# Keytoyze/Mug-Diffusion

Hardware: NVIDIA H100
Metric: denoising-steps/sec (higher is better)
Workload: dtype f32

## Files before the change

include/mugd.h:

```cpp
#ifndef MUGD_H
#define MUGD_H

#include <stdint.h>

#ifdef __cplusplus
extern "C" {
#endif

#define MUGD_ABI_VERSION 13

typedef struct mugd_handle mugd_handle;
typedef struct mugd_plan mugd_plan;

enum mugd_status {
    MUGD_OK = 0,
    MUGD_ERR_INVALID = 1,
    MUGD_ERR_CUDA = 2,
    MUGD_ERR_NO_DEVICE = 3,
    MUGD_ERR_OOM = 4
};

enum mugd_op_kind {
    MUGD_OP_GEMM = 1,
    MUGD_OP_GROUPNORM = 2,
// ... 66 lines not shown
} mugd_layernorm;

typedef struct mugd_attention {
    const float* q; int64_t ldq;
    const float* k; int64_t ldk;
    const float* v; int64_t ldv;
    float* o; int64_t ldo;
    const float* relpos;
    const float* cgain;
    int32_t B, H, D, Lq, Lk, pos_max; float scale;
} mugd_attention;

typedef struct mugd_s4conv {
    const float* u; int64_t ldu;
    const float* Kt;
    const float* D;
    float* y; int64_t ldy;
    int32_t B, L, H;
} mugd_s4conv;

typedef struct mugd_ddim_update {
    float* x;
    float* x_dup;
    const float* eps;
    const float* noise;
    float* pred_x0;
    const float* coef;
    const int32_t* step;
    int32_t S; int32_t n;
    int32_t cfg; float scale; float temperature;
} mugd_ddim_update;

typedef struct mugd_transpose {
    const float* in; float* out;
    int64_t ldi, ldo; int32_t B, C, L, to_nlc;
} mugd_transpose;

typedef struct mugd_copy2d {
    const float* src; int64_t lds; float* dst; int64_t ldd; int32_t rows, cols;
} mugd_copy2d;

typedef struct mugd_step_advance { int32_t* step; } mugd_step_advance;

typedef struct mugd_notes {
    const float* logits; int64_t ld;
    int32_t* count; int32_t* start_ms; int32_t* end_ms;
    double frame_ms;
    int32_t B, T, K;
} mugd_notes;

typedef struct mugd_embed {
    const float* table;
    const int32_t* ids;
    float* out;
    int32_t B, F, H, n_embed;
} mugd_embed;

typedef struct mugd_tf32_split { float* w_hi; float* lo; int64_t n; } mugd_tf32_split;

typedef struct mugd_posterior {
    const float* params;
    const float* noise;
    float *mean, *logvar, *std, *z;
    float scale;
    int32_t B, Z, L;
} mugd_posterior;

typedef struct mugd_groupnorm_var {
    mugd_groupnorm gn;
    const int32_t* valid;
} mugd_groupnorm_var;

typedef struct mugd_attention_var {
    mugd_attention attn;
    const int32_t* valid;
} mugd_attention_var;

typedef struct mugd_row_mask {
    float* x; int64_t ld;
    const int32_t* valid;
    int32_t B, L, cols, reserved_;
} mugd_row_mask;

typedef struct mugd_op {
    int32_t kind;
    int32_t tag;
    union {
        mugd_gemm gemm; mugd_groupnorm gn; mugd_layernorm ln; mugd_attention attn; mugd_s4conv s4;
        mugd_ddim_update ddim; mugd_transpose tr; mugd_copy2d cp; mugd_step_advance adv; mugd_notes notes;
        mugd_embed embed; mugd_tf32_split split; mugd_posterior post;
        mugd_groupnorm_var gnv; mugd_attention_var attnv; mugd_row_mask mask;
    } u;
} mugd_op;

int  mugd_abi_version(void);
const char* mugd_last_error(void);
int  mugd_create(int device, mugd_handle** out);
void mugd_destroy(mugd_handle* h);
int  mugd_device_info(mugd_handle* h, int32_t* sm_count, int32_t* cc_major, int32_t* cc_minor);
int  mugd_set_gemm_impl(mugd_handle* h, int impl);
int  mugd_set_pdl(int enabled);

int  mugd_op_run(mugd_handle* h, const mugd_op* op, void* stream);

int  mugd_plan_create(mugd_handle* h, const mugd_op* ops, int32_t n_ops, mugd_plan** out);
int  mugd_plan_run(mugd_plan* p, void* stream);
int  mugd_plan_capture(mugd_plan* p, void* stream);
int  mugd_plan_replay(mugd_plan* p, int32_t times, void* stream);
int  mugd_plan_launch_count(mugd_plan* p);
void mugd_plan_destroy(mugd_plan* p);

int  mugd_sample(mugd_plan* eval_plan, const mugd_op* tail, int32_t n_tail, int32_t n_steps, void* stream);

typedef struct mugd_stage {
    float* x; float* x_dup;
    const float* x0;
    const float* mask;
    const float* q_noise;
    const float* q_coef;
    const float* noise;
    float* noise_rows;
    int32_t B, C, L, reserved_;
} mugd_stage;
int  mugd_sample_staged(mugd_plan* eval_plan, const mugd_stage* stage, const mugd_op* tail, int32_t n_tail, int32_t n_steps,
                        void* stream);

typedef struct mugd_plms {
    mugd_ddim_update update;
    const float* eps;
    float* e_prime;
    float* hist;
    float* x_stash;
    int32_t cfg; float scale;
} mugd_plms;
int  mugd_sample_plms(mugd_plan* eval_plan, const mugd_plms* p, int32_t first_step, int32_t n_steps, void* stream);
int  mugd_plms_combine(const mugd_plms* p, int32_t step, int32_t heun, void* stream);

#define MUGD_MAX_STEPS 1000
typedef struct mugd_ddpm {
    float* x; float* x_dup;
    const float* eps;
    float* pred_x0;
    const float* noise;
    const float* coef;
    int32_t* step;
    int32_t T, B, C, L;
    int32_t cfg; float scale;
    int32_t clip;
    int32_t reserved_;
} mugd_ddpm;
int  mugd_sample_ddpm(mugd_plan* eval_plan, const mugd_ddpm* d, int32_t first_step, int32_t n_steps, void* stream);
int  mugd_ddpm_update(const mugd_ddpm* d, void* stream);

typedef struct mugd_dpm {
    float* x; float* x_dup;
    const float* eps;
    float* pred_x0;
    float* ring;
    const float* coef;
    int32_t* step;
    int32_t n, S;
    int32_t cfg; float scale;
} mugd_dpm;
int  mugd_sample_dpm(mugd_plan* eval_plan, const mugd_dpm* d, int32_t first_step, int32_t n_steps, void* stream);
int  mugd_dpm_update(const mugd_dpm* d, void* stream);

typedef struct mugd_dpm_ex {
    mugd_dpm dpm;
    const mugd_stage* stage;
    const int32_t* start;
    const float* order_coef;
    int32_t B, reserved_;
} mugd_dpm_ex;
int  mugd_sample_dpm_ex(mugd_plan* eval_plan, const mugd_dpm_ex* e, int32_t first_step, int32_t n_steps, void* stream);
// ... 130 lines not shown
```

mug_diffusion_b200/bundle.py:

```python
from __future__ import annotations

import argparse
import ctypes as C
import os
from typing import Dict, List, Optional, Tuple

import numpy as np
import torch

from . import lib as L_
from . import seeding
from .engine import OpList
from .runtime import Plan, _ptr
from .sampler import draw_step_noise, q_coef_table


def _save_plan(eng, ops: OpList, regions: List[L_.Region], path: str) -> Plan:
    pl = Plan(eng, ops)
    arr = (L_.Region * len(regions))(*regions)
    L_.check(eng.lib.mugd_plan_save(pl.handle, arr, len(regions), path.encode()), f"plan_save {path}")
    return pl


def export_bundle(model, inp: Dict[str, torch.Tensor], S: int, scale: float, out_dir: str, eta: float = 0.0, temperature: float = 1.0,
                  noise_dropout: float = 0.0, inpaint: Optional[Tuple[torch.Tensor, torch.Tensor]] = None,
                  seeds=None) -> Dict[str, torch.Tensor]:
    from .sampler import DDIMSampler

    os.makedirs(out_dir, exist_ok=True)
    eng = model.engine
    dev = eng.device
    cfg = eng.cfg
    B, Cz, Lz = inp["x_T"].shape
    if seeds is not None:
        if noise_dropout > 0.:
            raise ValueError("a seeded bundle draws no dropout mask")
        seeds = seeding.chart_seeds(seeds, B)
    cfg_on = scale != 1.0
    Beff = 2 * B if cfg_on else B
    sampler = DDIMSampler(model)
    sampler.make_schedule(S, ddim_eta=eta, verbose=False)
    ts = np.flip(sampler.ddim_timesteps)
    total = len(ts)

    with eng.lock:
        sess = eng.session(Beff, Lz, per_sample_t=False)
        dec = eng.decoder_session(B, Lz)
        T = inp["c"].shape[2]
        sess.set_ctx_tokens(T)
        seeded = None if seeds is None else seeding.ChartNoise(seeds, (B, Cz, Lz), dev)
        x_T = inp["x_T"] if seeded is None else seeded.draw(seeding.X_T, 0)
        st = dict(in_x=x_T.to(dev).contiguous(), in_c=inp["c"].to(dev).contiguous(), in_uc=inp["uc"].to(dev).contiguous(),
                  pred=torch.zeros(B * Lz * Cz, device=dev), out_z=torch.zeros(B, Cz, Lz, device=dev),
                  out_logits=torch.zeros(B, cfg.decoder.x_channels, dec.Lout, device=dev))
        w4 = [w.to(dev).contiguous() for w in list(inp["w"])[-cfg.unet.levels:]]
        for i, w in enumerate(w4):
            st[f"in_w{i}"] = w
        has_noise = bool(np.any(np.asarray(sampler.ddim_sigmas) != 0))
        staged = has_noise or inpaint is not None
        shape = (B, Cz, Lz)
        if has_noise:
            st["noise_rows"] = torch.zeros(B * Lz * Cz, device=dev)
            st["in_noise"] = torch.empty((total,) + shape, device=dev)
        if inpaint is not None:
            st["in_x0"] = inpaint[0].to(dev, torch.float32).contiguous()
            st["in_mask"] = inpaint[1].to(dev, torch.float32).expand(shape).contiguous()
            st["in_qnoise"] = torch.empty((total,) + shape, device=dev)
            qcoef = q_coef_table(model, ts)
            qcoef.tofile(os.path.join(out_dir, "stage_coef.bin"))
        randn_rows = {} if seeded is None else dict(seeded=seeded, first_draw=total - 1, draw_stride=-1)
        draw_step_noise(total, shape, st.get("in_x0"), st.get("in_qnoise"), has_noise, st.get("in_noise"), noise_dropout, dev,
                        **randn_rows)
        drawn = {} if seeded is None else {"in_x": (seeding.X_T, 0, 1, 1)}
        if seeded is not None:
            drawn.update({k: (p, total - 1, total, -1) for k, p in (("in_noise", seeding.STEP), ("in_qnoise", seeding.Q)) if k in st})
        sess.set_timestep_table(ts.copy())
        sess.set_ddim_schedule(sampler.ddim_alphas, sampler.ddim_alphas_prev, sampler.ddim_sigmas, sampler.ddim_sqrt_one_minus_alphas)

        tensors: Dict[str, torch.Tensor] = dict(weights=eng.weights, weights_lo=eng.weights_lo, arena=sess.arena_t, emb_table=sess.emb_table, temb=sess.temb,
                                                emb_h1=sess.emb_h1, emb_h2=sess.emb_h2, step=sess.step, coef=sess.coef, ctx=sess.ctx,
                                                tc_ws=eng.tc_ws, tc_counters=eng.tc_counters, dec_arena=dec.arena_t)
        for i, t in enumerate(sess.ctx_kv):
            tensors[f"ctx_kv{i}"] = t
        for i, (_, t) in enumerate(sorted(sess.s4_kt.items())):
            tensors[f"s4_kt{i}"] = t
        tensors.update(st)
        contents = {"weights", "weights_lo", "temb", "coef"} | {k for k in tensors if k.startswith("s4_kt")}
        inputs = {k for k in st if k.startswith("in_")}
        names = list(tensors)
        keep = [n.encode() for n in names]
        regions = [L_.Region(keep[i], _ptr(tensors[n]), tensors[n].numel() * tensors[n].element_size()) for i, n in enumerate(names)]

        tail = sess.ddim_tail(B, total, cfg_on, scale, temperature, _ptr(st["pred"]), _ptr(st["noise_rows"]) if has_noise else 0)
        stage = None
        if staged:
            stage = sess.ddim_stage(B, cfg_on, _ptr(st["noise_rows"]) if has_noise else 0)
            if has_noise:
                stage.noise = _ptr(st["in_noise"])
            if inpaint is not None:
                stage.x0, stage.mask, stage.q_noise = _ptr(st["in_x0"]), _ptr(st["in_mask"]), _ptr(st["in_qnoise"])
                stage.q_coef = qcoef.ctypes.data
        readz = OpList()
        readz.transpose(sess.xin.ptr, _ptr(st["out_z"]), sess.xin.ld, 0, B, Cz, Lz, False)
        dec_in = OpList()
        assert cfg.decoder.scale == 1.0, "bundle export assumes first-stage scale 1 (the shipped config)"
        dec_in.transpose(_ptr(st["out_z"]), dec.zin.ptr, 0, dec.zin.ld, B, cfg.decoder.z_channels, Lz, True)
        dec_out = OpList()
        dec_out.transpose(dec.logits.ptr, _ptr(st["out_logits"]), dec.logits.ld, 0, B, cfg.decoder.x_channels, dec.Lout, False)
        ctx_parts = [(_ptr(st["in_uc"]), B), (_ptr(st["in_c"]), B)] if cfg_on else [(_ptr(st["in_c"]), B)]
        seq = [("emb", sess.timestep_ops(total), "run"), ("ctx", sess.context_ops(ctx_parts, T), "run"),
               ("audio", sess.audio_ops([_ptr(w) for w in w4], cfg_on), "run"), ("loadx", sess.loadx_ops(_ptr(st["in_x"]), B, cfg_on), "run"),
               ("eval", None, "graph"), ("tail", tail, "tail"), ("readz", readz, "run"), ("dec_in", dec_in, "run"), ("dec", None, "graph"),
               ("dec_out", dec_out, "run")]
        plans = {}
        lines = ["mugd_bundle 1", f"# z_length {Lz} batch {B} guidance {scale} steps {total} (S={S})"]
        for n in names:
            t = tensors[n]
            nbytes = t.numel() * t.element_size()
            if (n in contents or n in inputs) and n not in drawn:
                t.detach().cpu().contiguous().numpy().tofile(os.path.join(out_dir, n + ".bin"))
                lines.append(f"region {n} {nbytes} file {n}.bin")
            else:
                lines.append(f"region {n} {nbytes} zero -")
        if seeded is not None:
            seeding.seed_array(seeds).tofile(os.path.join(out_dir, "seeds.bin"))
            lines.append(f"seeds seeds.bin {B}")
            for n, (purpose, first, count, stride) in drawn.items():
                lines.append(f"randn {n} {purpose} {first} {count} {stride} {B} {Cz * Lz}")
        for name, ops, mode in seq:
            path = os.path.join(out_dir, name + ".plan")
            if ops is None:
                pl = sess.plan if name == "eval" else dec.plan
                arr = (L_.Region * len(regions))(*regions)
                L_.check(eng.lib.mugd_plan_save(pl.handle, arr, len(regions), path.encode()), f"plan_save {name}")
            else:
                pl = _save_plan(eng, ops, regions, path)
            plans[name] = pl
            if mode == "tail":
                continue
            if name == "eval" and staged:
                for field in ("x", "x_dup", "x0", "mask", "q_noise", "noise", "noise_rows"):
                    ptr = getattr(stage, field)
                    if ptr:
                        region = next(n for n in names if 0 <= ptr - _ptr(tensors[n]) < tensors[n].numel() * tensors[n].element_size())
                        lines.append(f"stage {field} {region} {ptr - _ptr(tensors[region])}")
                lines.append(f"staged eval.plan tail.plan {total} {'stage_coef.bin' if inpaint is not None else '-'} {B} {Cz} {Lz}")
            elif name == "eval":
                lines.append(f"sample eval.plan tail.plan {total}")
            else:
                lines.append(f"plan {name}.plan {mode}")

        sess.set_step(0)
        for name in ("emb", "ctx", "audio", "loadx"):
            plans[name].run()
        sess.plan.launch(total, tail, stage)
        for name in ("readz", "dec_in"):
            plans[name].run()
        dec.plan.launch()
        plans["dec_out"].run()
        torch.cuda.synchronize()
        for n in ("out_z", "out_logits"):
            st[n].cpu().numpy().tofile(os.path.join(out_dir, n + ".expected.bin"))
            lines.append(f"expect {n} {st[n].numel() * 4} {n}.expected.bin")
        open(os.path.join(out_dir, "manifest.txt"), "w").write("\n".join(lines) + "\n")
        return dict(z=st["out_z"].clone(), logits=st["out_logits"].clone())


def main():
    from . import synth
    from .sampler import MugDiffusionB200
# ... 29 lines not shown
```

mug_diffusion_b200/csrc/api.cu:

```cuda
#include <stdarg.h>
#include <string.h>

#include <vector>

#include "common.cuh"

namespace mugd {

static thread_local char g_err[1024] = "";
bool g_use_pdl = true;

void set_error(const char* fmt, ...) {
    va_list ap;
    va_start(ap, fmt);
    vsnprintf(g_err, sizeof(g_err), fmt, ap);
    va_end(ap);
}

}

struct mugd_handle {
    mugd::DeviceInfo dev;
    int default_gemm_impl = MUGD_GEMM_SIMT;
};

struct mugd_plan {
    mugd_handle* h = nullptr;
    std::vector<mugd_op> ops;
    cudaGraph_t graph = nullptr;
    cudaGraphExec_t exec = nullptr;
    int launches = 0;
};

namespace mugd {

const std::vector<mugd_op>& plan_ops(const mugd_plan* p) { return p->ops; }
int plan_from_ops(mugd_handle* h, const mugd_op* ops, int32_t n, mugd_plan** out) { return mugd_plan_create(h, ops, n, out); }

static int dispatch(mugd_handle* h, const mugd_op& op, cudaStream_t st, int* launches, const mugd_gemm* next_tc = nullptr) {
    switch (op.kind) {
        case MUGD_OP_GEMM: return launch_gemm(h->dev, op.u.gemm, h->default_gemm_impl, next_tc, st, launches);
        case MUGD_OP_GROUPNORM: return launch_groupnorm(h->dev, op.u.gn, st, launches);
        case MUGD_OP_LAYERNORM: return launch_layernorm(h->dev, op.u.ln, st, launches);
        case MUGD_OP_ATTENTION: return launch_attention(h->dev, op.u.attn, st, launches);
        case MUGD_OP_S4CONV: return launch_s4conv(h->dev, op.u.s4, st, launches);
        case MUGD_OP_DDIM_UPDATE: return launch_ddim_update(h->dev, op.u.ddim, st, launches);
        case MUGD_OP_TRANSPOSE: return launch_transpose(h->dev, op.u.tr, st, launches);
        case MUGD_OP_COPY2D: return launch_copy2d(h->dev, op.u.cp, st, launches);
        case MUGD_OP_STEP_ADVANCE: return launch_step_advance(h->dev, op.u.adv, st, launches);
        case MUGD_OP_NOTES: return launch_notes(h->dev, op.u.notes, st, launches);
        case MUGD_OP_EMBED: return launch_embed(h->dev, op.u.embed, st, launches);
        case MUGD_OP_TF32_SPLIT: return launch_tf32_split(h->dev, op.u.split, st, launches);
        case MUGD_OP_POSTERIOR: return launch_posterior(h->dev, op.u.post, st, launches);
        case MUGD_OP_GROUPNORM_VAR: return launch_groupnorm_var(h->dev, op.u.gnv, st, launches);
        case MUGD_OP_ATTENTION_VAR: return launch_attention_var(h->dev, op.u.attnv, st, launches);
        case MUGD_OP_ROW_MASK: return launch_row_mask(h->dev, op.u.mask, st, launches);
        default:
            set_error("unknown op kind %d", op.kind);
            return MUGD_ERR_INVALID;
    }
}

template <typename Before, typename After>
static int run_steps(const mugd_plan* eval_plan, int32_t n_steps, int32_t* step, cudaStream_t st, Before before, After after) {
    mugd_step_advance adv;
    adv.step = step;
    for (int32_t k = 0; k < n_steps; ++k) {
        int rc = before(k);
        if (rc != MUGD_OK) return rc;
        MUGD_CHECK_CUDA(cudaGraphLaunch(eval_plan->exec, st));
        if ((rc = after(k)) != MUGD_OK) return rc;
        if (step && (rc = launch_step_advance(eval_plan->h->dev, adv, st, nullptr)) != MUGD_OK) return rc;
    }
    return MUGD_OK;
}

static int no_kernels(int32_t) { return MUGD_OK; }

template <typename Before>
static int run_tail_steps(const mugd_plan* eval_plan, const mugd_op* tail, int32_t n_tail, int32_t n_steps, cudaStream_t st,
                          Before before) {
    return run_steps(eval_plan, n_steps, nullptr, st, before, [&](int32_t) {
        for (int32_t k = 0; k < n_tail; ++k) {
            int rc = dispatch(eval_plan->h, tail[k], st, nullptr);
            if (rc != MUGD_OK) return rc;
        }
        return (int)MUGD_OK;
    });
}

static int run_dpm_steps(const mugd_plan* eval_plan, const mugd_dpm_ex& e, int32_t n_steps, cudaStream_t st) {
    return run_steps(
        eval_plan, n_steps, e.dpm.step, st, [&](int32_t k) { return e.stage ? launch_stage(*e.stage, k, st) : MUGD_OK; },
        [&](int32_t) { return launch_dpm_ex_update(e, st); });
}

static int check_step_range(const char* fn, int32_t first_step, int32_t n_steps, const char* total_name, int32_t total) {
    MUGD_REQUIRE(first_step >= 0 && n_steps >= 0 && (int64_t)first_step + n_steps <= total,
                 "%s: first_step=%d, n_steps=%d outside the %s=%d steps of the request", fn, first_step, n_steps, total_name, total);
    return MUGD_OK;
}

static int check_tail_rows(const char* fn, const char* what, int k, const mugd_ddim_update& d, const float* x, const float* x_dup,
                           int32_t B, int32_t C, int32_t L) {
    const int64_t n = (int64_t)B * C * L;
    MUGD_REQUIRE(d.x == x && d.x_dup == x_dup, "%s: tail op %d updates other rows than the %s's x / x_dup", fn, k, what);
    MUGD_REQUIRE(d.n == n, "%s: tail op %d updates n=%d elements, the %s B*C*L=%lld", fn, k, d.n, what, (long long)n);
    return MUGD_OK;
}

}

using namespace mugd;

extern "C" {

int mugd_abi_version(void) { return MUGD_ABI_VERSION; }

const char* mugd_last_error(void) { return g_err; }

int mugd_create(int device, mugd_handle** out) {
    MUGD_REQUIRE(out, "mugd_create: null out");
    *out = nullptr;
    int n = 0;
    cudaError_t e = cudaGetDeviceCount(&n);
    if (e != cudaSuccess || n <= 0 || device < 0 || device >= n) {
        set_error("mugd_create: no CUDA device %d (count=%d, %s). libmugd has no CPU fallback.", device, n,
                  e == cudaSuccess ? "ok" : cudaGetErrorString(e));
        return MUGD_ERR_NO_DEVICE;
    }
    cudaDeviceProp prop;
    MUGD_CHECK_CUDA(cudaGetDeviceProperties(&prop, device));
    if (prop.major != 9 || prop.minor != 0) {
        set_error("mugd_create: device %d is sm_%d%d; libmugd is built for sm_90a (H100) only", device, prop.major, prop.minor);
        return MUGD_ERR_NO_DEVICE;
    }
    MUGD_CHECK_CUDA(cudaSetDevice(device));
// ... 196 lines not shown
}

int mugd_sample_dpm_ex(mugd_plan* eval_plan, const mugd_dpm_ex* e, int32_t first_step, int32_t n_steps, void* stream) {
    MUGD_REQUIRE(e, "mugd_sample_dpm_ex: null descriptor");
    int rc = check_dpm_ex(*e, n_steps);
    if (rc != MUGD_OK) return rc;
    if ((rc = check_step_range("mugd_sample_dpm_ex", first_step, n_steps, "S", e->dpm.S)) != MUGD_OK) return rc;
    MUGD_REQUIRE(eval_plan && eval_plan->exec, "mugd_sample_dpm_ex: the evaluation plan must be captured (mugd_plan_capture)");
    return run_dpm_steps(eval_plan, *e, n_steps, (cudaStream_t)stream);
}

int mugd_sample_dpm_stop(mugd_plan* eval_plan, const mugd_dpm_stop* e, int32_t first_step, int32_t n_steps, void* stream) {
    MUGD_REQUIRE(e, "mugd_sample_dpm_stop: null descriptor");
    int rc = check_dpm_stop(*e);
    if (rc != MUGD_OK) return rc;
    if ((rc = check_step_range("mugd_sample_dpm_stop", first_step, n_steps, "S", e->dpm.S)) != MUGD_OK) return rc;
    MUGD_REQUIRE(eval_plan && eval_plan->exec, "mugd_sample_dpm_stop: the evaluation plan must be captured (mugd_plan_capture)");
    cudaStream_t st = (cudaStream_t)stream;
    return run_steps(eval_plan, n_steps, e->dpm.step, st, no_kernels, [&](int32_t) { return launch_dpm_stop_update(*e, st); });
}

int mugd_sample_unipc(mugd_plan* eval_plan, const mugd_unipc* u, int32_t first_step, int32_t n_steps, void* stream) {
    MUGD_REQUIRE(u, "mugd_sample_unipc: null descriptor");
    int rc = check_unipc(*u);
    if (rc != MUGD_OK) return rc;
    if ((rc = check_step_range("mugd_sample_unipc", first_step, n_steps, "S", u->dpm.S)) != MUGD_OK) return rc;
    MUGD_REQUIRE(eval_plan && eval_plan->exec, "mugd_sample_unipc: the evaluation plan must be captured (mugd_plan_capture)");
    cudaStream_t st = (cudaStream_t)stream;
    return run_steps(eval_plan, n_steps, u->dpm.step, st, no_kernels, [&](int32_t) { return launch_unipc_update(*u, st); });
}

int mugd_sample_unipc_ex(mugd_plan* eval_plan, const mugd_unipc_ex* e, int32_t first_step, int32_t n_steps, void* stream) {
    MUGD_REQUIRE(e, "mugd_sample_unipc_ex: null descriptor");
    int rc = check_unipc_ex(*e, n_steps);
    if (rc != MUGD_OK) return rc;
    if ((rc = check_step_range("mugd_sample_unipc_ex", first_step, n_steps, "S", e->unipc.dpm.S)) != MUGD_OK) return rc;
    MUGD_REQUIRE(eval_plan && eval_plan->exec, "mugd_sample_unipc_ex: the evaluation plan must be captured (mugd_plan_capture)");
    cudaStream_t st = (cudaStream_t)stream;
    return run_steps(
        eval_plan, n_steps, e->unipc.dpm.step, st, [&](int32_t k) { return e->stage ? launch_stage(*e->stage, k, st) : MUGD_OK; },
        [&](int32_t) { return launch_unipc_ex_update(*e, st); });
}

int mugd_sample_unipc_stop(mugd_plan* eval_plan, const mugd_unipc_stop* e, int32_t first_step, int32_t n_steps, void* stream) {
    MUGD_REQUIRE(e, "mugd_sample_unipc_stop: null descriptor");
    int rc = check_unipc_stop(*e);
    if (rc != MUGD_OK) return rc;
    if ((rc = check_step_range("mugd_sample_unipc_stop", first_step, n_steps, "S", e->unipc.dpm.S)) != MUGD_OK) return rc;
    MUGD_REQUIRE(eval_plan && eval_plan->exec, "mugd_sample_unipc_stop: the evaluation plan must be captured (mugd_plan_capture)");
    cudaStream_t st = (cudaStream_t)stream;
    return run_steps(eval_plan, n_steps, e->unipc.dpm.step, st, no_kernels, [&](int32_t) { return launch_unipc_stop_update(*e, st); });
}

int mugd_sample_join(mugd_plan* eval_plan, const mugd_join* join, const mugd_op* tail, int32_t n_tail, int32_t first_step,
                     int32_t n_steps, void* stream) {
    MUGD_REQUIRE(eval_plan && eval_plan->exec, "mugd_sample_join: the evaluation plan must be captured (mugd_plan_capture)");
    MUGD_REQUIRE(join, "mugd_sample_join: null join");
    MUGD_REQUIRE(n_tail >= 0 && (n_tail == 0 || tail), "mugd_sample_join: bad tail (n_tail=%d)", n_tail);
    const mugd_join& j = *join;
    int rc = check_join(j);
    if (rc != MUGD_OK) return rc;
    const mugd_ddim_update* upd = nullptr;
    for (int k = 0; k < n_tail; ++k) {
        if (tail[k].kind != MUGD_OP_DDIM_UPDATE) continue;
        MUGD_REQUIRE(!upd, "mugd_sample_join: the tail holds more than one DDIM update (op %d)", k);
        upd = &tail[k].u.ddim;
        if ((rc = check_tail_rows("mugd_sample_join", "join", k, *upd, j.x, j.x_dup, j.B, j.C, j.L)) != MUGD_OK) return rc;
        MUGD_REQUIRE(upd->step, "mugd_sample_join: tail op %d has no device step counter", k);
    }
    MUGD_REQUIRE(upd, "mugd_sample_join: the tail holds no DDIM update");
    if ((rc = check_step_range("mugd_sample_join", first_step, n_steps, "S", upd->S)) != MUGD_OK) return rc;
    cudaStream_t st = (cudaStream_t)stream;
    return run_tail_steps(eval_plan, tail, n_tail, n_steps, st, [&](int32_t) { return launch_join(j, upd->step, st); });
}

int mugd_abi_sizes(int32_t* out, int32_t n) {
    MUGD_REQUIRE(out && n >= 13, "abi_sizes: need room for 13 entries");
    out[0] = sizeof(mugd_op); out[1] = sizeof(mugd_gemm); out[2] = sizeof(mugd_groupnorm);
    out[3] = sizeof(mugd_layernorm); out[4] = sizeof(mugd_attention); out[5] = sizeof(mugd_s4conv);
    out[6] = sizeof(mugd_ddim_update); out[7] = sizeof(mugd_transpose); out[8] = sizeof(mugd_copy2d);
    out[9] = sizeof(mugd_notes); out[10] = sizeof(mugd_embed); out[11] = sizeof(mugd_tf32_split);
    out[12] = sizeof(mugd_posterior);
    if (n >= 16) { out[13] = sizeof(mugd_groupnorm_var); out[14] = sizeof(mugd_attention_var); out[15] = sizeof(mugd_row_mask); }
    return MUGD_OK;
}

int mugd_plan_ops(mugd_plan* p, const mugd_op** ops, int32_t* n_ops) {
    MUGD_REQUIRE(p && ops && n_ops, "plan_ops: bad arguments");
    *ops = p->ops.data();
    *n_ops = (int32_t)p->ops.size();
    return MUGD_OK;
}

int mugd_plan_launch_count(mugd_plan* p) { return p ? p->launches : 0; }

void mugd_plan_destroy(mugd_plan* p) {
    if (!p) return;
    if (p->exec) cudaGraphExecDestroy(p->exec);
    if (p->graph) cudaGraphDestroy(p->graph);
    delete p;
}

}
```

mug_diffusion_b200/csrc/common.cuh:

```cuda
#pragma once
#include <cuda_runtime.h>
#include <stdint.h>
#include <stdio.h>
#include <string.h>
#include <string>
#include <utility>

#include "../../include/mugd.h"

#if defined(__CUDA_ARCH__) && (__CUDA_ARCH__ != 900)
#error "libmugd is written for sm_90a (H100) only"
#endif

namespace mugd {

void set_error(const char* fmt, ...);

#define MUGD_CHECK_CUDA(expr)                                                             \
    do {                                                                                  \
        cudaError_t _e = (expr);                                                          \
        if (_e != cudaSuccess) {                                                          \
            ::mugd::set_error("%s:%d %s -> %s", __FILE__, __LINE__, #expr,                \
                              cudaGetErrorString(_e));                                    \
            return MUGD_ERR_CUDA;                                                         \
        }                                                                                 \
    } while (0)

#define MUGD_REQUIRE(cond, ...)                                                           \
    do {                                                                                  \
        if (!(cond)) {                                                                    \
            ::mugd::set_error(__VA_ARGS__);                                               \
            return MUGD_ERR_INVALID;                                                      \
        }                                                                                 \
    } while (0)

struct DeviceInfo {
    int device = 0;
    int sm_count = 132;
    int cc_major = 0, cc_minor = 0;
    int max_smem_optin = 0;
    int tc_single_pass = 0;
    int attention_impl = 1;
    int s4conv_impl = 0;
};

int launch_gemm(const DeviceInfo& dev, const mugd_gemm& g, int default_impl, const mugd_gemm* next, cudaStream_t st, int* launches);
bool gemm_runs_tc(const mugd_gemm& g, int default_impl);
int launch_groupnorm(const DeviceInfo& dev, const mugd_groupnorm& g, cudaStream_t st, int* launches);
int launch_layernorm(const DeviceInfo& dev, const mugd_layernorm& g, cudaStream_t st, int* launches);
int launch_attention(const DeviceInfo& dev, const mugd_attention& a, cudaStream_t st, int* launches);
int launch_s4conv(const DeviceInfo& dev, const mugd_s4conv& s, cudaStream_t st, int* launches);
int launch_ddim_update(const DeviceInfo& dev, const mugd_ddim_update& d, cudaStream_t st, int* launches);
int launch_transpose(const DeviceInfo& dev, const mugd_transpose& t, cudaStream_t st, int* launches);
int launch_copy2d(const DeviceInfo& dev, const mugd_copy2d& c, cudaStream_t st, int* launches);
int launch_step_advance(const DeviceInfo& dev, const mugd_step_advance& a, cudaStream_t st, int* launches);
int launch_notes(const DeviceInfo& dev, const mugd_notes& n, cudaStream_t st, int* launches);
int launch_embed(const DeviceInfo& dev, const mugd_embed& e, cudaStream_t st, int* launches);
int launch_tf32_split(const DeviceInfo& dev, const mugd_tf32_split& s, cudaStream_t st, int* launches);
int launch_posterior(const DeviceInfo& dev, const mugd_posterior& p, cudaStream_t st, int* launches);
int launch_groupnorm_var(const DeviceInfo& dev, const mugd_groupnorm_var& g, cudaStream_t st, int* launches);
int launch_attention_var(const DeviceInfo& dev, const mugd_attention_var& a, cudaStream_t st, int* launches);
int launch_row_mask(const DeviceInfo& dev, const mugd_row_mask& m, cudaStream_t st, int* launches);
int check_stage(const mugd_stage& s, int32_t n_steps);
int launch_stage(const mugd_stage& s, int32_t i, cudaStream_t st);
int check_plms(const mugd_plms& p);
int launch_plms_combine(const mugd_plms& p, int32_t step, int heun, cudaStream_t st);
int check_ddpm(const mugd_ddpm& d);
int launch_ddpm_update(const mugd_ddpm& d, int32_t k, cudaStream_t st);
int check_dpm(const mugd_dpm& d);
int launch_dpm_update(const mugd_dpm& d, cudaStream_t st);
int check_dpm_ex(const mugd_dpm_ex& e, int32_t n_steps);
int launch_dpm_ex_update(const mugd_dpm_ex& e, cudaStream_t st);
int check_dpm_stop(const mugd_dpm_stop& e);
int launch_dpm_stop_update(const mugd_dpm_stop& e, cudaStream_t st);
int check_unipc(const mugd_unipc& u);
int launch_unipc_update(const mugd_unipc& u, cudaStream_t st);
int check_unipc_ex(const mugd_unipc_ex& e, int32_t n_steps);
int launch_unipc_ex_update(const mugd_unipc_ex& e, cudaStream_t st);
int check_unipc_stop(const mugd_unipc_stop& e);
int launch_unipc_stop_update(const mugd_unipc_stop& e, cudaStream_t st);
int check_join(const mugd_join& j);
int launch_join(const mugd_join& j, const int32_t* step, cudaStream_t st);
int launch_gemm_tc(const DeviceInfo& dev, const mugd_gemm& g, const mugd_gemm* next, cudaStream_t st, int* launches);
bool gemm_tc_supported(const mugd_gemm& g);

inline int check_cfg(const char* who, int cfg) {
    MUGD_REQUIRE(cfg == 0 || cfg == 1, "%s: cfg=%d", who, cfg);
    return MUGD_OK;
}
inline int check_scale(const char* who, float scale) {
    MUGD_REQUIRE(isfinite(scale), "%s: scale is not finite", who);
    return MUGD_OK;
}
inline int check_x_dup(const char* who, const float* x_dup, int cfg) {
    MUGD_REQUIRE(!x_dup == !cfg, "%s: x_dup must be given exactly when cfg = 1 (the evaluation reads x in both halves)", who);
    return MUGD_OK;
}
inline int check_tile_grid(const char* who, int32_t B, int32_t C, int32_t L) {
    MUGD_REQUIRE(B > 0 && C > 0 && L > 0 && (int64_t)B * C * L <= INT32_MAX, "%s: bad shape B=%d C=%d L=%d", who, B, C, L);
    MUGD_REQUIRE(B <= 65535 && (C + 31) / 32 <= 65535, "%s: B=%d / C=%d too large for one launch", who, B, C);
    return MUGD_OK;
}

cudaError_t gemm_tc_allow_smem(int bytes);
cudaError_t attention_tc_allow_smem(int bytes);
cudaError_t attention_allow_smem(int bytes);
cudaError_t s4_allow_smem(int bytes);

extern bool g_use_pdl;

#ifdef __CUDACC__
template <typename... KArgs, typename... Args>
inline cudaError_t launch_k(void (*kernel)(KArgs...), dim3 grid, dim3 block, size_t smem, cudaStream_t st, Args&&... args) {
    cudaLaunchConfig_t cfg = {};
    cfg.gridDim = grid;
    cfg.blockDim = block;
    cfg.dynamicSmemBytes = smem;
    cfg.stream = st;
    cudaLaunchAttribute attr[1];
    attr[0].id = cudaLaunchAttributeProgrammaticStreamSerialization;
    attr[0].val.programmaticStreamSerializationAllowed = 1;
    cfg.attrs = attr;
    cfg.numAttrs = g_use_pdl ? 1 : 0;
    return cudaLaunchKernelEx(&cfg, kernel, std::forward<Args>(args)...);
}
template <typename... Kernels>
inline cudaError_t allow_dynamic_smem(int bytes, Kernels... kernels) {
    cudaError_t e = cudaSuccess;
    ((e = (e == cudaSuccess) ? cudaFuncSetAttribute(kernels, cudaFuncAttributeMaxDynamicSharedMemorySize, bytes) : e), ...);
    return e;
}
__device__ __forceinline__ void pdl_wait() { asm volatile("griddepcontrol.wait;" ::: "memory"); }

__device__ __forceinline__ float cfg_eps(const float* eps, int64_t i, int64_t n, int cfg, float scale) {
    if (!cfg) return eps[i];
    const float eu = eps[i], ec = eps[n + i];
    return __fadd_rn(eu, __fmul_rn(scale, __fsub_rn(ec, eu)));
}

__device__ __forceinline__ void load_ncl_tile(float (&tile)[32][33], const float* in, int c0, int l0, int C, int L) {
    const int tx = threadIdx.x & 31, ty = threadIdx.x >> 5;
#pragma unroll
    for (int r = ty; r < 32; r += 8) {
// ... 35 lines not shown
```

mug_diffusion_b200/csrc/gemm_tc.cu:

```cuda
#include "gemm_tc.cuh"

namespace mugd {

template <int BN, int EPI>
__global__ void __launch_bounds__(TC_THREADS, 1)
gemm_tc_kernel(const __grid_constant__ CUtensorMap tmA, const __grid_constant__ CUtensorMap tmA1,
               const __grid_constant__ CUtensorMap tmA2, const __grid_constant__ CUtensorMap tmB, const __grid_constant__ CUtensorMap tmWhi,
               const __grid_constant__ CUtensorMap tmWlo, const __grid_constant__ TcParams p) {
    extern __shared__ uint8_t smem_raw[];
    const uint32_t base = (smem_u32(smem_raw) + 1023u) & ~1023u;
    const TcBars<BN> B(base);
    TC_STAMP(p, 0, blockIdx.x == 0 && blockIdx.y == 0 && blockIdx.z == 0);
    if (threadIdx.x < 32) {
        B.init_parallel((int)threadIdx.x);
    } else if (threadIdx.x < 38) {
        const CUtensorMap* m = threadIdx.x == 32 ? &tmA : threadIdx.x == 33 ? &tmA1 : threadIdx.x == 34 ? &tmA2
                             : threadIdx.x == 35 ? &tmB : threadIdx.x == 36 ? &tmWhi : &tmWlo;
        asm volatile("prefetch.tensormap [%0];" ::"l"(reinterpret_cast<uint64_t>(m)) : "memory");
    }
    __syncthreads();
    TC_STAMP(p, 1, blockIdx.x == 0 && blockIdx.y == 0 && blockIdx.z == 0);
    gemm_tc_tile<BN, EPI>(&tmA, &tmA1, &tmA2, &tmB, &tmWhi, &tmWlo, p, blockIdx.x, blockIdx.y, blockIdx.z, base);
}

template <int BN, int EPI>
__global__ void __launch_bounds__(TC_THREADS)
gemm_tc_reduce_kernel(const __grid_constant__ TcParams p) {
    tc_reduce<BN, EPI>(p, blockIdx.x);
}

#ifdef MUGD_TC_TIMELINE
static long long* g_tc_dbg = nullptr;
#endif
static float g_tc_kstep128 = 0.55f;
static float g_tc_split = 3.0f;
static int g_tc_force_bn = 0;

static bool tc_shape_ok(const mugd_gemm& g) {
    if (!(g.conv_mode == MUGD_CONV_NONE || g.conv_mode == MUGD_CONV_SAME || g.conv_mode == MUGD_CONV_DOWN ||
          g.conv_mode == MUGD_CONV_TAPS)) return false;
    if (g.conv_mode == MUGD_CONV_DOWN && g.Lout < 2) return false;
    if (g.K2 % TC_BK != 0 || (g.K2 > 0 && g.conv_mode == MUGD_CONV_DOWN)) return false;
    return g.K % TC_BK == 0 && g.N >= 16 && g.N % 4 == 0;
}

bool gemm_tc_supported(const mugd_gemm& g) {
    if (!tc_shape_ok(g)) return false;
    if (!g.W_hi || !g.W_lo) return false;
    if (g.lda % 4 != 0 || !aligned16(g.A) || !aligned16(g.W_hi) || !aligned16(g.W_lo)) return false;
    if (g.K2 > 0 && (!g.A2 || g.lda2 % 4 != 0 || !aligned16(g.A2))) return false;
    return true;
}

static int tc_validate_fusions(const mugd_gemm& g) {
    if (g.row_moments)
        MUGD_REQUIRE(g.act == MUGD_ACT_NONE && g.gate == MUGD_GATE_NONE && !g.ln_stats && (reinterpret_cast<uintptr_t>(g.row_moments) & 15u) == 0,
                     "gemm: row_moments needs act == gate == NONE, no folded LayerNorm and a 16-byte aligned buffer");
    if (g.ln_stats) {
        MUGD_REQUIRE(g.ln_colsum && aligned16(g.ln_colsum) && (reinterpret_cast<uintptr_t>(g.ln_stats) & 15u) == 0 && g.taps == 1 && g.K2 == 0 &&
                         g.act == MUGD_ACT_NONE && (g.gate == MUGD_GATE_NONE || g.gate == MUGD_GATE_GEGLU) && !g.rowvec,
                     "gemm: folded LayerNorm needs a single-source Linear with act NONE and gate NONE/GEGLU");
    }
    return MUGD_OK;
}

TcGeometry tc_geometry(const mugd_gemm& g, int sm_count, int forced_split) {
    TcGeometry t = {};
    TcParams::Hot& h = t.hot;
    t.BN = (g.N >= 128) ? 128 : 64;
    if (g.conv_mode == MUGD_CONV_NONE) { h.Lrows = g.M; h.Bs = 1; }
    else { h.Lrows = g.Lout; h.Bs = g.M / g.Lout; }
    if (h.Lrows >= TC_BM) {
        h.box_l = TC_BM; h.box_b = 1;
        h.tiles_per_sample = (h.Lrows + TC_BM - 1) / TC_BM;
        t.gy = h.tiles_per_sample * h.Bs;
    } else {
        h.box_l = h.Lrows;
        h.box_b = TC_BM / h.Lrows;
        if (h.box_b > h.Bs) h.box_b = h.Bs;
        h.tiles_per_sample = 1;
        t.gy = (h.Bs + h.box_b - 1) / h.box_b;
    }
    h.kblocks = g.K / TC_BK;
    h.it_main = g.taps * h.kblocks;
    h.total_it = h.it_main + g.K2 / TC_BK;
    int splits = 1;
    float best = 1e30f;
    static const int cands[2] = {64, 128};
    for (int cand = 0; cand < 2; ++cand) {
        const int bn = cands[cand];
        if (bn > 64 && g.N < bn) continue;
        if (bn == 64 && g.N >= 128 && g_tc_force_bn != 64) continue;
        if (g_tc_force_bn && bn != g_tc_force_bn && !(g_tc_force_bn > g.N && bn == 64)) continue;
        const int gx = (g.N + bn - 1) / bn;
        const int tiles = gx * t.gy;
        const float kstep = bn == 128 ? g_tc_kstep128 : 0.4f;
        const int sp_max = forced_split > 0 ? forced_split : (tiles < sm_count ? 16 : 1);
        for (int sp = forced_split > 0 ? forced_split : 1; sp <= sp_max && sp <= h.total_it; ++sp) {
            const int per = (h.total_it + sp - 1) / sp;
            if (forced_split <= 0 && sp > 1 && per < 2) break;
            if (forced_split <= 0 && sp > 1 && tiles * sp > 2 * sm_count) break;
            const int waves = (tiles * sp + sm_count - 1) / sm_count;
            const float est = waves * (1.0f + kstep * per) + (sp > 1 ? g_tc_split : 0.0f);
            if (est < best - 0.25f) { best = est; splits = sp; t.BN = bn; }
        }
    }
    h.gx = (g.N + t.BN - 1) / t.BN;
    if (splits > h.total_it) splits = h.total_it;
    if (splits < 1) splits = 1;
    h.splits = splits;
    h.it_base = h.total_it / splits;
    h.it_rem = h.total_it % splits;
    h.conv_mode = g.conv_mode;
    h.tap_shift = g.tap_shift;
    h.tap_dilation = g.tap_dilation;
    t.ws_floats = splits > 1 ? (int64_t)h.gx * t.gy * splits * TC_BM * t.BN : 0;
    return t;
}

int tc_plan(const DeviceInfo& dev, const mugd_gemm& g, const mugd_gemm* next, TcPlanned* out) {
    MUGD_REQUIRE(gemm_tc_supported(g), "gemm_tc: unsupported shape/operands");
    int rc = tc_validate_fusions(g);
    if (rc != MUGD_OK) return rc;
    const TcGeometry t = tc_geometry(g, dev.sm_count, g.split_k);
    const TcParams::Hot& h = t.hot;
    if (h.splits > 1) {
        MUGD_REQUIRE(g.workspace, "gemm_tc: split-K needs a workspace");
        MUGD_REQUIRE(g.workspace_bytes >= t.ws_floats * 4, "gemm_tc: workspace too small (%lld < %lld)", (long long)g.workspace_bytes,
                     (long long)t.ws_floats * 4);
    }
    const cuuint32_t a_box[3] = {(cuuint32_t)TC_BK, (cuuint32_t)h.box_l, (cuuint32_t)h.box_b};
    for (int tap = 0; tap < 3; ++tap) {
        if (tap > 0 && g.conv_mode != MUGD_CONV_DOWN) { out->maps[tap] = out->maps[0]; continue; }
        const bool down = g.conv_mode == MUGD_CONV_DOWN;
        const cuuint64_t rows = down ? (cuuint64_t)(h.Lrows - (tap == 2 ? 1 : 0)) : (cuuint64_t)h.Lrows;
        const cuuint64_t sample_rows = down ? (cuuint64_t)g.Lin : (cuuint64_t)h.Lrows;
        const cuuint64_t dims[3] = {(cuuint64_t)g.K, rows, (cuuint64_t)h.Bs};
        const cuuint64_t strides[2] = {(cuuint64_t)g.lda * 4 * (down ? 2 : 1), sample_rows * (cuuint64_t)g.lda * 4};
        rc = encode_f32_tma(&out->maps[tap], g.A + (down ? (int64_t)tap * g.lda : 0), 3, dims, strides, a_box, CU_TENSOR_MAP_L2_PROMOTION_L2_128B,
                            "gemm_tc A");
        if (rc != MUGD_OK) return rc;
    }
    if (g.K2 > 0) {
        const cuuint64_t dims[3] = {(cuuint64_t)g.K2, (cuuint64_t)h.Lrows, (cuuint64_t)h.Bs};
        const cuuint64_t strides[2] = {(cuuint64_t)g.lda2 * 4, (cuuint64_t)h.Lrows * (cuuint64_t)g.lda2 * 4};
        rc = encode_f32_tma(&out->maps[3], g.A2, 3, dims, strides, a_box, CU_TENSOR_MAP_L2_PROMOTION_L2_128B, "gemm_tc A2");
        if (rc != MUGD_OK) return rc;
    } else {
        out->maps[3] = out->maps[0];
    }
    const cuuint64_t ktot = (cuuint64_t)g.taps * g.K + g.K2;
    const cuuint64_t w_dims[2] = {ktot, (cuuint64_t)g.N};
    const cuuint64_t w_strides[1] = {ktot * 4};
    const cuuint32_t w_box[2] = {(cuuint32_t)TC_BK, (cuuint32_t)t.BN};
    for (int w = 0; w < 2; ++w) {
        rc = encode_f32_tma(&out->maps[4 + w], w == 0 ? g.W_hi : g.W_lo, 2, w_dims, w_strides, w_box, CU_TENSOR_MAP_L2_PROMOTION_L2_256B,
                            "gemm_tc W");
        if (rc != MUGD_OK) return rc;
    }
    TcParams& p = out->p;
    memset(&p, 0, sizeof(p));
    p.hot = h;
    p.hot.single_pass = dev.tc_single_pass ? 1 : 0;
    p.g = g;
    p.ws = (float*)g.workspace;
    p.gy = t.gy;
    p.ln_invK = 1.0 / (double)g.K;
    if (next) {
        p.pf_hi = next->W_hi;
        p.pf_lo = p.hot.single_pass ? nullptr : next->W_lo;
        p.pf_bytes = (int64_t)next->N * ((int64_t)next->taps * next->K + next->K2) * 4;
    }
#ifdef MUGD_TC_TIMELINE
    p.dbg = g_tc_dbg;
#endif
    out->BN = t.BN;
    return MUGD_OK;
}

template <int BN, int EPI>
static int tc_launch(const TcPlanned& pl, cudaStream_t st) {
    const TcParams& p = pl.p;
    const TcParams::Hot& h = p.hot;
// ... 108 lines not shown
```

mug_diffusion_b200/csrc/norm.cu:

```cuda
#include "common.cuh"

namespace mugd {

constexpr int GN_THREADS = 256;
constexpr int GN_MAXV = 32;

__device__ __forceinline__ void gn_block_stats(double s, double ss, double inv_n, float eps, float& mean, float& rstd) {
    __shared__ double red[2][GN_THREADS / 32];
    s = warp_sum(s);
    ss = warp_sum(ss);
    const int warp = threadIdx.x >> 5, lane = threadIdx.x & 31;
    if (lane == 0) { red[0][warp] = s; red[1][warp] = ss; }
    __syncthreads();
    double ts = 0.0, tss = 0.0;
#pragma unroll
    for (int w = 0; w < GN_THREADS / 32; ++w) { ts += red[0][w]; tss += red[1][w]; }
    const double m = ts * inv_n;
    const double var = tss * inv_n - m * m;
    const float v = fmaxf((float)var, 0.f) + eps;
    float r = rsqrtf(v);
    r = r * (1.5f - 0.5f * v * r * r);
    mean = (float)m;
    rstd = r;
}

template <int NV>
__device__ __forceinline__ void gn_reg_body(const float* __restrict__ x, int64_t ldx, float* __restrict__ y, int64_t ldy,
                                            const float* __restrict__ gamma, const float* __restrict__ beta,
                                            int L, int Lv, int C, int G, float eps, int silu) {
    const int g = blockIdx.x, b = blockIdx.y;
    const int cg = C / G;
    const int q = cg >> 2;
    const int total = Lv * q;
    const double inv_n = 1.0 / ((double)Lv * cg);
    const float* xb = x + (int64_t)b * L * ldx + (int64_t)g * cg;
    float* yb = y + (int64_t)b * L * ldy + (int64_t)g * cg;
    float4 v[NV];
#pragma unroll
    for (int u = 0; u < NV; ++u) {
        const int i = (int)threadIdx.x + u * GN_THREADS;
        v[u] = make_float4(0.f, 0.f, 0.f, 0.f);
        if (i < total) {
            const int row = i / q, qq = i - row * q;
            v[u] = ld_f4(xb + (int64_t)row * ldx + qq * 4);
        }
    }
    double s = 0.0, ss = 0.0;
#pragma unroll
    for (int u = 0; u < NV; ++u) {
        s += (double)v[u].x + (double)v[u].y + (double)v[u].z + (double)v[u].w;
        ss += (double)v[u].x * v[u].x + (double)v[u].y * v[u].y + (double)v[u].z * v[u].z + (double)v[u].w * v[u].w;
    }
    const float* gm = gamma + g * cg;
    const float* bt = beta + g * cg;
    constexpr bool PRE = NV <= 8;
    float4 gav[PRE ? NV : 1], bev[PRE ? NV : 1];
    if constexpr (PRE) {
#pragma unroll
        for (int u = 0; u < NV; ++u) {
            const int i = (int)threadIdx.x + u * GN_THREADS;
            const int qq = i < total ? i % q : 0;
            gav[u] = ld_f4(gm + qq * 4);
            bev[u] = ld_f4(bt + qq * 4);
        }
    }
    float mean, rstd;
    gn_block_stats(s, ss, inv_n, eps, mean, rstd);
#pragma unroll
    for (int u = 0; u < NV; ++u) {
        const int i = (int)threadIdx.x + u * GN_THREADS;
        if (i < total) {
            const int row = i / q, qq = i - row * q;
            float4 ga, be;
            if constexpr (PRE) { ga = gav[u]; be = bev[u]; }
            else { ga = ld_f4(gm + qq * 4); be = ld_f4(bt + qq * 4); }
            float4 o;
            o.x = (v[u].x - mean) * rstd * ga.x + be.x;
            o.y = (v[u].y - mean) * rstd * ga.y + be.y;
            o.z = (v[u].z - mean) * rstd * ga.z + be.z;
            o.w = (v[u].w - mean) * rstd * ga.w + be.w;
            if (silu) { o.x = silu_f(o.x); o.y = silu_f(o.y); o.z = silu_f(o.z); o.w = silu_f(o.w); }
            st_f4(yb + (int64_t)row * ldy + qq * 4, o);
        }
    }
}

template <int NV>
__global__ void __launch_bounds__(GN_THREADS)
groupnorm_silu_reg_kernel(const float* __restrict__ x, int64_t ldx, float* __restrict__ y, int64_t ldy,
                          const float* __restrict__ gamma, const float* __restrict__ beta,
                          int L, int C, int G, float eps, int silu) {
    pdl_wait();
    gn_reg_body<NV>(x, ldx, y, ldy, gamma, beta, L, L, C, G, eps, silu);
}

__device__ __forceinline__ void gn_body(const float* __restrict__ x, int64_t ldx, float* __restrict__ y, int64_t ldy,
                                        const float* __restrict__ gamma, const float* __restrict__ beta,
                                        int L, int Lv, int C, int G, float eps, int silu) {
    const int g = blockIdx.x, b = blockIdx.y;
    const int cg = C / G;
    const int q = cg >> 2;
    const int total = Lv * q;
    const double inv_n = 1.0 / ((double)Lv * cg);
    const float* xb = x + (int64_t)b * L * ldx + (int64_t)g * cg;
    float* yb = y + (int64_t)b * L * ldy + (int64_t)g * cg;

    double s = 0.0, ss = 0.0;
    for (int i = threadIdx.x; i < total; i += GN_THREADS) {
        const int row = i / q, qq = i - row * q;
        const float4 v = ld_f4(xb + (int64_t)row * ldx + qq * 4);
        s += (double)v.x + (double)v.y + (double)v.z + (double)v.w;
        ss += (double)v.x * v.x + (double)v.y * v.y + (double)v.z * v.z + (double)v.w * v.w;
    }
    float mean, rstd;
    gn_block_stats(s, ss, inv_n, eps, mean, rstd);
    const float* gm = gamma + g * cg;
    const float* bt = beta + g * cg;
    for (int i = threadIdx.x; i < total; i += GN_THREADS) {
        const int row = i / q, qq = i - row * q;
        const float4 v = ld_f4(xb + (int64_t)row * ldx + qq * 4);
        const float4 ga = ld_f4(gm + qq * 4);
        const float4 be = ld_f4(bt + qq * 4);
        float4 o;
        o.x = (v.x - mean) * rstd * ga.x + be.x;
        o.y = (v.y - mean) * rstd * ga.y + be.y;
        o.z = (v.z - mean) * rstd * ga.z + be.z;
        o.w = (v.w - mean) * rstd * ga.w + be.w;
        if (silu) { o.x = silu_f(o.x); o.y = silu_f(o.y); o.z = silu_f(o.z); o.w = silu_f(o.w); }
        st_f4(yb + (int64_t)row * ldy + qq * 4, o);
    }
}

__global__ void __launch_bounds__(GN_THREADS)
groupnorm_silu_kernel(const float* __restrict__ x, int64_t ldx, float* __restrict__ y, int64_t ldy,
                      const float* __restrict__ gamma, const float* __restrict__ beta,
                      int L, int C, int G, float eps, int silu) {
    pdl_wait();
    gn_body(x, ldx, y, ldy, gamma, beta, L, L, C, G, eps, silu);
}

__device__ __forceinline__ int gn_valid_rows(const int32_t* valid, int L) { return min(max(valid[blockIdx.y], 0), L); }

__device__ __forceinline__ void gn_zero_tail(float* y, int64_t ldy, int L, int Lv, int C, int G) {
    const int g = blockIdx.x, b = blockIdx.y;
    const int q = (C / G) >> 2;
    float* yb = y + ((int64_t)b * L + Lv) * ldy + (int64_t)g * (C / G);
    const float4 z = make_float4(0.f, 0.f, 0.f, 0.f);
    for (int i = threadIdx.x; i < (L - Lv) * q; i += GN_THREADS) {
        const int row = i / q, qq = i - row * q;
        st_f4(yb + (int64_t)row * ldy + qq * 4, z);
    }
}

template <int NV>
__global__ void __launch_bounds__(GN_THREADS)
groupnorm_silu_reg_var_kernel(const float* __restrict__ x, int64_t ldx, float* __restrict__ y, int64_t ldy,
                              const float* __restrict__ gamma, const float* __restrict__ beta,
                              int L, int C, int G, float eps, int silu, const int32_t* __restrict__ valid) {
    pdl_wait();
    const int Lv = gn_valid_rows(valid, L);
    gn_reg_body<NV>(x, ldx, y, ldy, gamma, beta, L, Lv, C, G, eps, silu);
    gn_zero_tail(y, ldy, L, Lv, C, G);
}

__global__ void __launch_bounds__(GN_THREADS)
groupnorm_silu_var_kernel(const float* __restrict__ x, int64_t ldx, float* __restrict__ y, int64_t ldy,
                          const float* __restrict__ gamma, const float* __restrict__ beta,
                          int L, int C, int G, float eps, int silu, const int32_t* __restrict__ valid) {
    pdl_wait();
    const int Lv = gn_valid_rows(valid, L);
    gn_body(x, ldx, y, ldy, gamma, beta, L, Lv, C, G, eps, silu);
    gn_zero_tail(y, ldy, L, Lv, C, G);
}

static int check_groupnorm(const mugd_groupnorm& g) {
    MUGD_REQUIRE(g.B > 0 && g.L > 0 && g.C > 0 && g.G > 0, "groupnorm: empty shape B=%d L=%d C=%d G=%d", g.B, g.L, g.C, g.G);
    MUGD_REQUIRE(g.C % g.G == 0 && (g.C / g.G) % 4 == 0, "groupnorm: C/G must be a multiple of 4 (C=%d G=%d)", g.C, g.G);
    MUGD_REQUIRE(g.ldx % 4 == 0 && g.ldy % 4 == 0 && aligned16(g.x) && aligned16(g.y) && aligned16(g.gamma) && aligned16(g.beta),
                 "groupnorm: operands must be 16-byte aligned with ld %% 4 == 0");
    MUGD_REQUIRE(g.ldx >= g.C && g.ldy >= g.C, "groupnorm: leading dimension smaller than C");
    return MUGD_OK;
}

int launch_groupnorm(const DeviceInfo&, const mugd_groupnorm& g, cudaStream_t st, int* launches) {
    const int rc = check_groupnorm(g);
    if (rc != MUGD_OK) return rc;
    dim3 grid(g.G, g.B);
    const int per_thread = (g.L * (g.C / g.G / 4) + GN_THREADS - 1) / GN_THREADS;
#define GN_GO(K) MUGD_CHECK_CUDA(launch_k(K, grid, dim3(GN_THREADS), 0, st, g.x, g.ldx, g.y, g.ldy, g.gamma, g.beta, g.L, g.C, g.G, g.eps, g.silu))
    if (per_thread <= 2) GN_GO(groupnorm_silu_reg_kernel<2>);
    else if (per_thread <= 4) GN_GO(groupnorm_silu_reg_kernel<4>);
    else if (per_thread <= 8) GN_GO(groupnorm_silu_reg_kernel<8>);
    else if (per_thread <= 16) GN_GO(groupnorm_silu_reg_kernel<16>);
    else if (per_thread <= GN_MAXV) GN_GO(groupnorm_silu_reg_kernel<GN_MAXV>);
    else GN_GO(groupnorm_silu_kernel);
#undef GN_GO
    if (launches) *launches += 1;
    return MUGD_OK;
}

int launch_groupnorm_var(const DeviceInfo&, const mugd_groupnorm_var& v, cudaStream_t st, int* launches) {
    const mugd_groupnorm& g = v.gn;
    int rc = check_groupnorm(g);
    if (rc != MUGD_OK) return rc;
    MUGD_REQUIRE(v.valid, "groupnorm_var: valid lengths missing");
    dim3 grid(g.G, g.B);
    const int per_thread = (g.L * (g.C / g.G / 4) + GN_THREADS - 1) / GN_THREADS;
#define GN_GO(K) MUGD_CHECK_CUDA(launch_k(K, grid, dim3(GN_THREADS), 0, st, g.x, g.ldx, g.y, g.ldy, g.gamma, g.beta, g.L, g.C, g.G, g.eps, g.silu, v.valid))
    if (per_thread <= 2) GN_GO(groupnorm_silu_reg_var_kernel<2>);
    else if (per_thread <= 4) GN_GO(groupnorm_silu_reg_var_kernel<4>);
    else if (per_thread <= 8) GN_GO(groupnorm_silu_reg_var_kernel<8>);
    else if (per_thread <= 16) GN_GO(groupnorm_silu_reg_var_kernel<16>);
    else if (per_thread <= GN_MAXV) GN_GO(groupnorm_silu_reg_var_kernel<GN_MAXV>);
    else GN_GO(groupnorm_silu_var_kernel);
#undef GN_GO
    if (launches) *launches += 1;
    return MUGD_OK;
}

constexpr int LN_WARPS = 8;
constexpr int LN_MAXQ = 8;

__global__ void __launch_bounds__(LN_WARPS * 32)
layernorm_kernel(const float* __restrict__ x, int64_t ldx, float* __restrict__ y, int64_t ldy,
                 const float* __restrict__ gamma, const float* __restrict__ beta, int rows, int C, float eps) {
    pdl_wait();
    const int row = blockIdx.x * LN_WARPS + (threadIdx.x >> 5);
    if (row >= rows) return;
    const int lane = threadIdx.x & 31;
    const int nq = C >> 2;
    const float* xr = x + (int64_t)row * ldx;
    float4 v[LN_MAXQ];
    float s = 0.f;
#pragma unroll
    for (int i = 0; i < LN_MAXQ; ++i) {
        const int qi = lane + i * 32;
        if (qi < nq) {
            v[i] = ld_f4(xr + qi * 4);
            s += (v[i].x + v[i].y) + (v[i].z + v[i].w);
        } else {
            v[i] = make_float4(0.f, 0.f, 0.f, 0.f);
        }
    }
    const float mean = warp_sum(s) / (float)C;
    float ss = 0.f;
#pragma unroll
    for (int i = 0; i < LN_MAXQ; ++i) {
        const int qi = lane + i * 32;
        if (qi < nq) {
            const float a = v[i].x - mean, b = v[i].y - mean, c = v[i].z - mean, d = v[i].w - mean;
            ss += (a * a + b * b) + (c * c + d * d);
        }
    }
    const float rstd = rsqrtf(warp_sum(ss) / (float)C + eps);
    float* yr = y + (int64_t)row * ldy;
#pragma unroll
    for (int i = 0; i < LN_MAXQ; ++i) {
        const int qi = lane + i * 32;
        if (qi < nq) {
            const float4 ga = ld_f4(gamma + qi * 4), be = ld_f4(beta + qi * 4);
            float4 o;
            o.x = (v[i].x - mean) * rstd * ga.x + be.x;
            o.y = (v[i].y - mean) * rstd * ga.y + be.y;
            o.z = (v[i].z - mean) * rstd * ga.z + be.z;
            o.w = (v[i].w - mean) * rstd * ga.w + be.w;
            st_f4(yr + qi * 4, o);
        }
    }
}

int launch_layernorm(const DeviceInfo&, const mugd_layernorm& g, cudaStream_t st, int* launches) {
    MUGD_REQUIRE(g.rows > 0 && g.C > 0, "layernorm: empty shape");
    MUGD_REQUIRE(g.C % 4 == 0 && g.C <= LN_MAXQ * 128, "layernorm: C=%d must be a multiple of 4 and <= %d", g.C, LN_MAXQ * 128);
    MUGD_REQUIRE(g.ldx % 4 == 0 && g.ldy % 4 == 0 && aligned16(g.x) && aligned16(g.y) && aligned16(g.gamma) && aligned16(g.beta),
                 "layernorm: operands must be 16-byte aligned with ld %% 4 == 0");
    MUGD_REQUIRE(g.ldx >= g.C && g.ldy >= g.C, "layernorm: leading dimension smaller than C");
    const int blocks = (g.rows + LN_WARPS - 1) / LN_WARPS;
    MUGD_CHECK_CUDA(launch_k(layernorm_kernel, dim3(blocks), dim3(LN_WARPS * 32), 0, st, g.x, g.ldx, g.y, g.ldy, g.gamma, g.beta, g.rows,
                             g.C, g.eps));
    if (launches) *launches += 1;
    return MUGD_OK;
}

}
```

mug_diffusion_b200/engine.py:

```python
from __future__ import annotations

import ctypes as C
from dataclasses import dataclass
from typing import Dict, List, Optional, Sequence, Tuple

import numpy as np
import torch

from . import lib as L_
from .config import DecoderConfig, EncoderConfig, ModelConfig, UNetConfig
from .dpm_solver import MAX_STEPS
from .netspec import RES_LAYERS, Block, decoder_layout, encoder_layout, unet_layout
from .packer import WeightBlob, pack_model

GN_EPS = 1e-6
LN_EPS = 1e-5
CTX_TOKENS_MAX = 64


@dataclass
class View:
    ptr: int
    ld: int
    rows: int
    cols: int

    def c(self, c0: int, c1: int) -> "View":
        assert 0 <= c0 < c1 <= self.cols, (c0, c1, self.cols)
        return View(self.ptr + 4 * c0, self.ld, self.rows, c1 - c0)

    def r(self, r0: int, r1: int) -> "View":
        assert 0 <= r0 < r1 <= self.rows
        return View(self.ptr + 4 * r0 * self.ld, self.ld, r1 - r0, self.cols)


class Arena:

    def __init__(self, base: int = 0, capacity: Optional[int] = None):
        self.base = base
        self.capacity = capacity
        self.top = 0
        self.high = 0

    def alloc(self, rows: int, cols: int) -> View:
        n = rows * cols * 4
        start = (self.top + 255) // 256 * 256
        self.top = start + n
        self.high = max(self.high, self.top)
        if self.capacity is not None:
            assert self.top <= self.capacity, "arena overflow"
        return View(self.base + start, cols, rows, cols)

    def mark(self) -> int:
        return self.top

    def release(self, mark: int):
        self.top = mark


class OpList:
    def __init__(self, tc_map: Optional[Dict[int, Tuple[int, int]]] = None, valid: Optional[Dict[int, int]] = None):
        self.ops: List[L_.Op] = []
        self.tc_map = tc_map or {}
        self.valid = valid or {}

    def add(self, kind: int, desc, tag: int = 0):
        self.ops.append(L_.make_op(kind, desc, tag))

    def array(self):
        arr = (L_.Op * len(self.ops))(*self.ops)
        return arr

    def gemm(self, A: View, W: int, N: int, K: int, out: View, *, bias: int = 0, taps: int = 1,
             mode: int = L_.CONV_NONE, Lin: int = 0, Lout: int = 0, act: int = L_.ACT_NONE,
             gate: int = L_.GATE_NONE, residual: Optional[View] = None, rowvec: int = 0,
             rowvec_b_stride: int = 0, rowvec_step_stride: int = 0, step: int = 0, impl: int = L_.GEMM_AUTO,
             W_hi: int = 0, W_lo: int = 0, split_k: int = 0, tap_shift: int = 0, dilation: int = 1, tag: int = 0,
             A2: Optional[View] = None, ln: Optional[Tuple[int, int, float]] = None) -> int:
        g = L_.Gemm()
        M = out.rows
        g.A, g.lda = A.ptr, A.ld
        if not W_hi and W in self.tc_map:
            W_hi, W_lo = self.tc_map[W]
        g.W, g.W_hi, g.W_lo, g.bias = W, W_hi or None, W_lo or None, bias or None
        g.split_k = split_k
        g.tap_shift = tap_shift
        g.tap_dilation = dilation
        g.rowvec, g.rowvec_b_stride, g.rowvec_step_stride = rowvec or None, rowvec_b_stride, rowvec_step_stride
        g.step = step or None
        if residual is not None:
            g.residual, g.ldr = residual.ptr, residual.ld
        if A2 is not None:
            assert A2.rows == out.rows, (A2.rows, out.rows)
            g.A2, g.lda2, g.K2 = A2.ptr, A2.ld, A2.cols
        g.C, g.ldc = out.ptr, out.ld
        g.M, g.N, g.K = M, N, K
        g.taps, g.conv_mode = taps, mode
        g.Lout = Lout or M
        g.Lin = Lin or g.Lout
        g.act, g.gate, g.impl = act, gate, impl
        if ln is not None:
            g.ln_stats, g.ln_colsum, g.ln_eps = ln[0], ln[1], float(ln[2])
        nout = N // 2 if gate else N
        assert out.cols == nout, (out.cols, nout)
        assert A.cols == K, (A.cols, K)
        self.add(L_.OP_GEMM, g, tag)
        return len(self.ops) - 1

    def can_deliver_row_moments(self, i: int) -> bool:
        op = self.ops[i]
        if op.kind != L_.OP_GEMM:
            return False
        g = op.u.gemm
        tc = bool(g.W_hi) and g.K % 32 == 0 and g.K2 % 32 == 0 and g.N >= 16 and g.impl != L_.GEMM_SIMT and g.conv_mode != L_.CONV_UP
        return tc and g.act == L_.ACT_NONE and g.gate == L_.GATE_NONE and not g.ln_stats and not g.row_moments

    def groupnorm(self, x: View, y: View, gamma: int, beta: int, B: int, Lrows: int, G: int, silu: bool, tag: int = 0) -> int:
        d = L_.GroupNorm()
        d.x, d.ldx, d.y, d.ldy = x.ptr, x.ld, y.ptr, y.ld
        d.gamma, d.beta = gamma, beta
        d.B, d.L, d.C, d.G = B, Lrows, x.cols, G
        d.eps, d.silu = GN_EPS, int(silu)
        assert x.rows == B * Lrows and y.cols == x.cols
        if Lrows in self.valid:
            v = L_.GroupNormVar()
            v.gn, v.valid = d, self.valid[Lrows]
            self.add(L_.OP_GROUPNORM_VAR, v, tag)
        else:
            self.add(L_.OP_GROUPNORM, d, tag)
        return len(self.ops) - 1

    def row_mask(self, x: View, B: int, Lrows: int, tag: int = 0):
        assert x.rows == B * Lrows
        d = L_.RowMask()
        d.x, d.ld, d.valid = x.ptr, x.ld, self.valid[Lrows]
        d.B, d.L, d.cols = B, Lrows, x.cols
        self.add(L_.OP_ROW_MASK, d, tag)

    def layernorm(self, x: View, y: View, gamma: int, beta: int, tag: int = 0):
        d = L_.LayerNorm()
        d.x, d.ldx, d.y, d.ldy = x.ptr, x.ld, y.ptr, y.ld
        d.gamma, d.beta = gamma, beta
        d.rows, d.C, d.eps = x.rows, x.cols, LN_EPS
        self.add(L_.OP_LAYERNORM, d, tag)
        return len(self.ops) - 1

    def attention(self, q: View, k: View, v: View, o: View, relpos: int, cgain: int, B: int, H: int, Lq: int,
                  Lk: int, pos_max: int, tag: int = 0, self_attn: bool = False):
        d = L_.Attention()
        D = q.cols // H
        d.q, d.ldq, d.k, d.ldk, d.v, d.ldv, d.o, d.ldo = q.ptr, q.ld, k.ptr, k.ld, v.ptr, v.ld, o.ptr, o.ld
        d.relpos, d.cgain = relpos, cgain
        d.B, d.H, d.D, d.Lq, d.Lk, d.pos_max = B, H, D, Lq, Lk, pos_max
        d.scale = float(D) ** -0.5
        if self_attn and Lq in self.valid:
            v = L_.AttentionVar()
            v.attn, v.valid = d, self.valid[Lq]
            self.add(L_.OP_ATTENTION_VAR, v, tag)
        else:
            self.add(L_.OP_ATTENTION, d, tag)

    def s4conv(self, u: View, Kt: int, Dp: int, y: View, B: int, Lrows: int, tag: int = 0):
        d = L_.S4Conv()
        d.u, d.ldu, d.Kt, d.D, d.y, d.ldy = u.ptr, u.ld, Kt, Dp, y.ptr, y.ld
        d.B, d.L, d.H = B, Lrows, u.cols
        self.add(L_.OP_S4CONV, d, tag)

    def transpose(self, inp: int, out: int, ldi: int, ldo: int, B: int, Cc: int, Lrows: int, to_nlc: bool, tag: int = 0):
        d = L_.Transpose()
        d.inp, d.out, d.ldi, d.ldo = inp, out, ldi, ldo
        d.B, d.C, d.L, d.to_nlc = B, Cc, Lrows, int(to_nlc)
        self.add(L_.OP_TRANSPOSE, d, tag)

    def copy2d(self, src: View, dst: View, tag: int = 0):
        d = L_.Copy2D()
        assert src.rows == dst.rows and src.cols == dst.cols
        d.src, d.lds, d.dst, d.ldd, d.rows, d.cols = src.ptr, src.ld, dst.ptr, dst.ld, src.rows, src.cols
        self.add(L_.OP_COPY2D, d, tag)


def emit_upsample_conv(ops: "OpList", blob: WeightBlob, wfn, prefix: str, x: View, out: View, Lin: int, cin: int, cout: int, tag: int):
    idx = []
    if (prefix + "conv.up_even.weight") in blob.entries:
        for parity, name, shift in ((0, "conv.up_even.weight", -1), (1, "conv.up_odd.weight", 0)):
            dst = View(out.ptr + 4 * parity * out.ld, 2 * out.ld, x.rows, out.cols)
            idx.append(ops.gemm(x, wfn(prefix + name), cout, cin, dst, bias=wfn(prefix + "conv.bias"), taps=2, mode=L_.CONV_TAPS,
                                Lin=Lin, Lout=Lin, tap_shift=shift, tag=tag))
    else:
        idx.append(ops.gemm(x, wfn(prefix + "conv.weight"), cout, cin, out, bias=wfn(prefix + "conv.bias"), taps=3, mode=L_.CONV_UP,
                            Lin=Lin, Lout=2 * Lin, tag=tag))
    return idx


def tc_weight_map(blob: WeightBlob, wbase: int, lo_base: Optional[int] = None) -> Dict[int, Tuple[int, int]]:
    if lo_base is None:
        lo_base = wbase + 4 * blob.numel
    return {wbase + 4 * off: (wbase + 4 * off, lo_base + 4 * lo) for _, off, _, lo in blob.tc}


TAG_RES, TAG_ATTN, TAG_S4, TAG_UPDOWN, TAG_IO = 1, 2, 3, 4, 5


def emit_res(ops: OpList, arena: Arena, wfn, b: Block, x: View, out: View, B: int, Lr: int, G: int, **emb):
    norm1, conv1, norm2, conv2, _ = RES_LAYERS[b.kind]
    p = b.prefix
    m = arena.mark()
    t1 = arena.alloc(x.rows, b.cin)
    ops.groupnorm(x, t1, wfn(p + norm1 + "weight"), wfn(p + norm1 + "bias"), B, Lr, G, True, TAG_RES)
    t2 = arena.alloc(x.rows, b.cout)
    ops.gemm(t1, wfn(p + conv1 + "weight"), b.cout, b.cin, t2, bias=wfn(p + conv1 + "bias"), taps=3, mode=L_.CONV_SAME, Lin=Lr, Lout=Lr,
             tag=TAG_RES, **emb)
    t3 = arena.alloc(x.rows, b.cout)
    ops.groupnorm(t2, t3, wfn(p + norm2 + "weight"), wfn(p + norm2 + "bias"), B, Lr, G, True, TAG_RES)
    if b.has_skip_conv:
        ops.gemm(t3, wfn(p + "out_skip.weight"), b.cout, b.cout, out, bias=wfn(p + "out_skip.bias"), taps=3, mode=L_.CONV_SAME,
                 Lin=Lr, Lout=Lr, A2=x, tag=TAG_RES)
    else:
        ops.gemm(t3, wfn(p + conv2 + "weight"), b.cout, b.cout, out, bias=wfn(p + conv2 + "bias"), taps=3, mode=L_.CONV_SAME,
                 Lin=Lr, Lout=Lr, residual=x, tag=TAG_RES)
    arena.release(m)


class UNetCompiler:

    def __init__(self, cfg: UNetConfig, blob: WeightBlob, wbase: int, tc_map: Optional[Dict[int, Tuple[int, int]]] = None,
                 prefix: str = "model.unet_model."):
        self.cfg, self.blob, self.wbase, self.prefix = cfg, blob, wbase, prefix
        self.tc_map = tc_weight_map(blob, wbase) if tc_map is None else tc_map
        self.lay = unet_layout(cfg, prefix)

    def w(self, name: str) -> int:
        return self.wbase + 4 * self.blob.offset(name)

    def compile(self, arena: Arena, Beff: int, Lz: int, ext: Dict[str, int], per_sample_t: bool, fold_ln: Optional[bool] = None,
                valid: Optional[Sequence[int]] = None) -> dict:
        cfg = self.cfg
        nlev = cfg.levels
        assert Lz % (1 << (nlev - 1)) == 0 and (Lz >> (nlev - 1)) % 4 == 0, "z_length must be a multiple of 32"
        rows = [Beff * (Lz >> l) for l in range(nlev)]
        lens = [Lz >> l for l in range(nlev)]
        if valid is not None:
            assert len(valid) == nlev, (len(valid), nlev)
        ops = OpList(self.tc_map, None if valid is None else {lens[l]: int(valid[l]) for l in range(nlev)})
        ragged = valid is not None
        mc = cfg.model_channels
        G = cfg.gn_groups
        if fold_ln is None:
            fold_ln = rows[0] < 8192
        fuse_ln = fold_ln and any(k.endswith("qkv_ln.weight") for k in self.blob.entries)

        lvl_of_ds = {1 << l: l for l in range(nlev)}
        ln_rows = sum(3 * rows[lvl_of_ds[b.ds]] for b in self.lay.blocks() if b.kind == "attn")
        stat_doubles = ln_rows * 2 if fuse_ln else 0
        stat_floats = (2 * stat_doubles + 63) // 64 * 64
        live = arena.alloc(1, stat_floats) if fuse_ln else None
        zeros = arena.alloc(1, stat_floats) if fuse_ln else None
        stat_top = [0]

        def stat_alloc(n_doubles: int) -> int:
            o = stat_top[0]
            stat_top[0] += (n_doubles + 1) // 2 * 2
            assert stat_top[0] <= stat_doubles, "row-moment block overflow"
            return live.ptr + 8 * o

        if fuse_ln:
            ops.copy2d(zeros, live, TAG_IO)

        xin = arena.alloc(rows[0], cfg.in_channels)
        eps = arena.alloc(rows[0], cfg.out_channels)
        ctx_tokens = ext["ctx_tokens"]
        down_cat = []
        ch = mc
        ch_in_level = []
        for l in range(nlev):
            ch_in_level.append(ch)
            down_cat.append(arena.alloc(rows[l], ch + cfg.audio_channels[l]))
            ch = cfg.channel_mult[l] * mc
        up_blocks = [e for e in self.lay.output if not isinstance(e, tuple)]
        up_cat: List[View] = []
        up_parts: List[Tuple[int, int, int]] = []
        skip_ch = list(self.lay.skip_channels)
        ch = cfg.channel_mult[-1] * mc
        bi = 0
        for level in reversed(range(nlev)):
            for i in range(cfg.num_res_blocks + 1):
                ich = skip_ch.pop()
                ca = cfg.audio_channels[level] if i == 0 else 0
                up_cat.append(arena.alloc(rows[level], ch + ca + ich))
                up_parts.append((ch, ca, ich))
                assert up_blocks[bi][0].cin == ch + ca + ich, (up_blocks[bi][0].cin, ch, ca, ich)
                ch = cfg.channel_mult[level] * mc
                bi += 1
        n_skips = len(self.lay.skip_channels)
        skip_home: List[View] = [None] * n_skips
        for k in range(n_skips):
            ub = n_skips - 1 - k
            ch_h, ca, ich = up_parts[ub]
            assert ich == self.lay.skip_channels[k]
            skip_home[k] = up_cat[ub].c(ch_h + ca, ch_h + ca + ich)
        audio_slots: List[Tuple[int, View]] = []
        for l in range(nlev):
            audio_slots.append((l, down_cat[l].c(ch_in_level[l], ch_in_level[l] + cfg.audio_channels[l])))
        bi = 0
        for level in reversed(range(nlev)):
            ch_h, ca, ich = up_parts[bi]
            audio_slots.append((level, up_cat[bi].c(ch_h, ch_h + ca)))
            bi += cfg.num_res_blocks + 1

        emb_total = self.blob.meta["emb_total"]
        emb_off = self.blob.meta["emb_offsets"]
        E = ext["emb_table"]
        step = ext["step"]

        gemm = ops.gemm

        def copy(src: View, dst: View, tag: int):
            ops.copy2d(src, dst, tag)

        def mask(x: View, lvl: int, tag: int):
            if ragged:
                ops.row_mask(x, Beff, lens[lvl], tag)

        def groupnorm(x: View, y: View, gamma: int, beta: int, Lr: int, silu: bool, tag: int):
            ops.groupnorm(x, y, gamma, beta, Beff, Lr, G, silu, tag)

        emb_row = dict(rowvec_b_stride=emb_total) if per_sample_t else dict(rowvec_step_stride=emb_total, step=step)
        attn_index = [0]

        def emit_attn(b: Block, x: View, out: View, lvl: int):
            Lr, Cc, H = lens[lvl], b.cin, b.heads
            m = arena.mark()
            p = b.prefix
            t = p + "transformer_blocks.0."
            kv = ext["ctx_kv"][attn_index[0]]
            attn_index[0] += 1
            g = arena.alloc(x.rows, Cc)
            groupnorm(x, g, self.w(p + "norm.weight"), self.w(p + "norm.bias"), Lr, False, TAG_ATTN)
            h0 = arena.alloc(x.rows, Cc)
            i_h0 = gemm(g, self.w(p + "proj_in.weight"), Cc, Cc, h0, bias=self.w(p + "proj_in.bias"), Lout=Lr, tag=TAG_ATTN)

            def normed_linear(src: View, i_src: int, norm: str, lin: str, N: int, dst: View, gate: int = L_.GATE_NONE, has_bias: bool = False):
                if fuse_ln and ops.can_deliver_row_moments(i_src):
                    lv = stat_alloc(src.rows * 2)
                    ops.ops[i_src].u.gemm.row_moments = lv
                    gemm(src, self.w(t + lin + "_ln.weight"), N, Cc, dst, bias=self.w(t + lin + "_ln.bias"), gate=gate, Lout=Lr,
                         ln=(lv, self.w(t + lin + "_ln.colsum"), LN_EPS), tag=TAG_ATTN)
                else:
                    n = arena.alloc(src.rows, Cc)
                    ops.layernorm(src, n, self.w(t + norm + ".weight"), self.w(t + norm + ".bias"), TAG_ATTN)
                    gemm(n, self.w(t + lin + ".weight"), N, Cc, dst, bias=self.w(t + lin + ".bias") if has_bias else 0, gate=gate,
                         Lout=Lr, tag=TAG_ATTN)

            qkv = arena.alloc(x.rows, 3 * Cc)
            normed_linear(h0, i_h0, "norm1", "attn1.qkv", 3 * Cc, qkv)
            ao = arena.alloc(x.rows, Cc)
            ops.attention(qkv.c(0, Cc), qkv.c(Cc, 2 * Cc), qkv.c(2 * Cc, 3 * Cc), ao,
                          self.w(t + "attn1.relative_position_embedding"), self.w(t + "attn1.C_embedding"),
                          Beff, H, Lr, Lr, cfg.pos_max, TAG_ATTN, self_attn=True)
            h1 = arena.alloc(x.rows, Cc)
            i_h1 = gemm(ao, self.w(t + "attn1.to_out.0.weight"), Cc, Cc, h1, bias=self.w(t + "attn1.to_out.0.bias"),
                        residual=h0, Lout=Lr, tag=TAG_ATTN)
            q2 = arena.alloc(x.rows, Cc)
            normed_linear(h1, i_h1, "norm2", "attn2.to_q", Cc, q2)
            ops.attention(q2, kv.c(0, Cc), kv.c(Cc, 2 * Cc), ao,
                          self.w(t + "attn2.relative_position_embedding"), self.w(t + "attn2.C_embedding"),
                          Beff, H, Lr, ctx_tokens, cfg.pos_max, TAG_ATTN)
            h2 = h0
            i_h2 = gemm(ao, self.w(t + "attn2.to_out.0.weight"), Cc, Cc, h2, bias=self.w(t + "attn2.to_out.0.bias"),
                        residual=h1, Lout=Lr, tag=TAG_ATTN)
            ff = arena.alloc(x.rows, 4 * Cc)
            normed_linear(h2, i_h2, "norm3", "ff.net.0.proj", 8 * Cc, ff, gate=L_.GATE_GEGLU, has_bias=True)
            gemm(ff, self.w(p + "ff_out.weight"), Cc, 4 * Cc, out, bias=self.w(p + "ff_out.bias"), residual=x, Lout=Lr,
                 A2=h2, tag=TAG_ATTN)
            arena.release(m)

        def emit_s4(b: Block, x: View, out: View, lvl: int):
            Lr, Hc = lens[lvl], b.cin
            m = arena.mark()
            p = b.prefix
            s_ = p + "s4_model."
            g = arena.alloc(x.rows, Hc)
            groupnorm(x, g, self.w(p + "norm.weight"), self.w(p + "norm.bias"), Lr, False, TAG_S4)
            y = arena.alloc(x.rows, Hc)
            ops.s4conv(g, ext["s4_kt"][p].ptr, self.w(s_ + "D"), y, Beff, Lr, TAG_S4)
            z = g
            gemm(y, self.w(s_ + "output_linear.0.weight"), 2 * Hc, Hc, z, bias=self.w(s_ + "output_linear.0.bias"),
                 gate=L_.GATE_GLU, Lout=Lr, tag=TAG_S4)
            mask(z, lvl, TAG_S4)
            gemm(z, self.w(p + "out_layer.weight"), Hc, Hc, out, bias=self.w(p + "out_layer.bias"), taps=3,
                 mode=L_.CONV_SAME, Lin=Lr, Lout=Lr, residual=x, tag=TAG_S4)
            arena.release(m)

        def run_blocks(blocks: List[Block], x: View, final_out: Optional[View], lvl: int) -> Tuple[View, int]:
            cur = x
            for j, b in enumerate(blocks):
                last = j == len(blocks) - 1
                if b.kind == "up":
                    tgt_rows = rows[lvl - 1]
                    out = final_out if (last and final_out is not None) else arena.alloc(tgt_rows, b.cout)
                    mask(cur, lvl, TAG_UPDOWN)
                    emit_upsample_conv(ops, self.blob, self.w, b.prefix, cur, out, lens[lvl], b.cin, b.cout, TAG_UPDOWN)
                    lvl -= 1
                    cur = out
                    continue
                out = final_out if (last and final_out is not None) else arena.alloc(cur.rows, b.cout)
                if b.kind == "res":
                    emit_res(ops, arena, self.w, b, cur, out, Beff, lens[lvl], G, rowvec=E + 4 * emb_off[b.prefix], **emb_row)
                elif b.kind == "attn":
                    emit_attn(b, cur, out, lvl)
                elif b.kind == "s4":
                    emit_s4(b, cur, out, lvl)
                else:
                    raise ValueError(b.kind)
                cur = out
            return cur, lvl

        if ragged:
            mask(xin, 0, TAG_IO)
            for l, view in audio_slots:
                mask(view, l, TAG_IO)

        k = 0
        lvl = 0
        h: Optional[View] = None
        for entry in self.lay.input:
            if isinstance(entry, tuple):
                h = down_cat[lvl]
                continue
            b0 = entry[0]
            if b0.kind == "conv_in":
                dst = down_cat[0].c(0, mc)
                gemm(xin, self.w(b0.prefix + "weight"), b0.cout, b0.cin, dst, bias=self.w(b0.prefix + "bias"), taps=3,
                     mode=L_.CONV_SAME, Lin=lens[0], Lout=lens[0], tag=TAG_IO)
                copy(dst, skip_home[k], TAG_IO)
                k += 1
                h = dst
            elif b0.kind == "down":
                dst = down_cat[lvl + 1].c(0, b0.cout)
                mask(h, lvl, TAG_UPDOWN)
                gemm(h, self.w(b0.prefix + "conv.weight"), b0.cout, b0.cin, dst, bias=self.w(b0.prefix + "conv.bias"),
                     taps=3, mode=L_.CONV_DOWN, Lin=lens[lvl], Lout=lens[lvl + 1], tag=TAG_UPDOWN)
                copy(dst, skip_home[k], TAG_UPDOWN)
                k += 1
                lvl += 1
                h = dst
            else:
                h, lvl = run_blocks(entry, h, skip_home[k], lvl)
                k += 1
        assert k == n_skips and lvl == nlev - 1

        h, lvl = run_blocks(self.lay.middle, h, up_cat[0].c(0, up_parts[0][0]), lvl)

        ub = 0
        final = arena.alloc(rows[0], mc)
        for entry in self.lay.output:
            if isinstance(entry, tuple):
                continue
            if ub + 1 < len(up_cat):
                nxt = up_cat[ub + 1].c(0, up_parts[ub + 1][0])
            else:
                nxt = final
            h, lvl = run_blocks(entry, up_cat[ub], nxt, lvl)
            ub += 1
        assert lvl == 0

        ob = self.lay.out
        m = arena.mark()
        t = arena.alloc(rows[0], mc)
        groupnorm(final, t, self.w(ob.prefix + "0.weight"), self.w(ob.prefix + "0.bias"), lens[0], True, TAG_IO)
        gemm(t, self.w(ob.prefix + "2.weight"), ob.cout, ob.cin, eps, bias=self.w(ob.prefix + "2.bias"), taps=3,
             mode=L_.CONV_SAME, Lin=lens[0], Lout=lens[0], tag=TAG_IO)
        arena.release(m)
        return dict(ops=ops, xin=xin, eps=eps, audio_slots=audio_slots, ln_folded=fuse_ln)


class DecoderCompiler:

    def __init__(self, cfg: DecoderConfig, blob: WeightBlob, wbase: int, tc_map: Optional[Dict[int, Tuple[int, int]]] = None,
                 prefix: str = "model.first_stage_model.decoder."):
        self.cfg, self.blob, self.wbase, self.prefix = cfg, blob, wbase, prefix
        self.tc_map = tc_weight_map(blob, wbase) if tc_map is None else tc_map
        self.seq = self.layout(cfg, prefix)

    layout = staticmethod(decoder_layout)

    def w(self, name: str) -> int:
        return self.wbase + 4 * self.blob.offset(name)

    def compile(self, arena: Arena, B: int, Lz: int, valid: Optional[Dict[int, int]] = None) -> dict:
        cfg = self.cfg
        ops = OpList(self.tc_map, None if valid is None else {Lz * m: int(p) for m, p in valid.items()})
        ragged = valid is not None
        G = cfg.num_groups
        first = self.seq[0]
        inp = arena.alloc(B * Lz * first.mul, first.cin)
        cur = inp
        out_view = None
        for b in self.seq:
            Lr = Lz * b.mul
            p = b.prefix
            if ragged and b.kind in ("dec_conv_in", "up", "down"):
                ops.row_mask(cur, B, Lr, TAG_IO if b.kind == "dec_conv_in" else TAG_UPDOWN)
            if b.kind == "dec_conv_in":
                o = arena.alloc(B * Lr, b.cout)
                ops.gemm(cur, self.w(p + "weight"), b.cout, b.cin, o, bias=self.w(p + "bias"), taps=3, mode=L_.CONV_SAME,
                         Lin=Lr, Lout=Lr, tag=TAG_IO)
                cur = o
            elif b.kind == "dec_res":
                o = arena.alloc(B * Lr, b.cout)
                emit_res(ops, arena, self.w, b, cur, o, B, Lr, G)
                cur = o
            elif b.kind == "up":
                o = arena.alloc(B * Lr * 2, b.cout)
                emit_upsample_conv(ops, self.blob, self.w, p, cur, o, Lr, b.cin, b.cout, TAG_UPDOWN)
                cur = o
            elif b.kind == "down":
                o = arena.alloc(B * Lr // 2, b.cout)
                ops.gemm(cur, self.w(p + "conv.weight"), b.cout, b.cin, o, bias=self.w(p + "conv.bias"), taps=3, mode=L_.CONV_DOWN,
                         Lin=Lr, Lout=Lr // 2, tag=TAG_UPDOWN)
                cur = o
            elif b.kind == "dec_out":
                t = arena.alloc(B * Lr, b.cin)
                ops.groupnorm(cur, t, self.w(p + "norm_out.weight"), self.w(p + "norm_out.bias"), B, Lr, G, True, TAG_IO)
                out_view = arena.alloc(B * Lr, b.cout)
                ops.gemm(t, self.w(p + "conv_out.weight"), b.cout, b.cin, out_view, bias=self.w(p + "conv_out.bias"), taps=3,
                         mode=L_.CONV_SAME, Lin=Lr, Lout=Lr, tag=TAG_IO)
                if ragged:
                    ops.row_mask(out_view, B, Lr, TAG_IO)
            else:
                raise ValueError(b.kind)
        return dict(ops=ops, inp=inp, out=out_view, Lout=Lz * self.seq[-1].mul)


class EncoderCompiler(DecoderCompiler):

    def __init__(self, cfg: EncoderConfig, blob: WeightBlob, wbase: int, tc_map: Optional[Dict[int, Tuple[int, int]]] = None,
                 prefix: str = "model.first_stage_model.encoder."):
        super().__init__(cfg, blob, wbase, tc_map, prefix)

    layout = staticmethod(encoder_layout)
```

mug_diffusion_b200/lib.py:

```python
from __future__ import annotations

import ctypes as C
import os
from typing import Optional

HERE = os.path.dirname(os.path.abspath(__file__))
LIB_PATH = os.environ.get("MUGD_LIB") or os.path.join(HERE, "libmugd.so")

(OP_GEMM, OP_GROUPNORM, OP_LAYERNORM, OP_ATTENTION, OP_S4CONV, OP_DDIM_UPDATE, OP_TRANSPOSE, OP_COPY2D, OP_STEP_ADVANCE, OP_NOTES, OP_EMBED,
 OP_TF32_SPLIT, OP_POSTERIOR) = range(1, 14)
OP_GROUPNORM_VAR, OP_ATTENTION_VAR, OP_ROW_MASK = 14, 15, 16
CONV_NONE, CONV_SAME, CONV_DOWN, CONV_UP, CONV_TAPS = range(5)
ACT_NONE, ACT_SILU, ACT_GELU = range(3)
GATE_NONE, GATE_GEGLU, GATE_GLU = range(3)
GEMM_AUTO, GEMM_SIMT, GEMM_TC = range(3)
ABI_VERSION = 13

_f = C.c_void_p


class Gemm(C.Structure):
    _fields_ = [("A", _f), ("lda", C.c_int64), ("W", _f), ("W_hi", _f), ("W_lo", _f), ("bias", _f), ("rowvec", _f),
                ("rowvec_b_stride", C.c_int64), ("rowvec_step_stride", C.c_int64), ("step", _f),
                ("residual", _f), ("ldr", C.c_int64), ("C", _f), ("ldc", C.c_int64),
# ... 49 lines not shown
class StepAdvance(C.Structure):
    _fields_ = [("step", _f)]


class Notes(C.Structure):
    _fields_ = [("logits", _f), ("ld", C.c_int64), ("count", _f), ("start_ms", _f), ("end_ms", _f), ("frame_ms", C.c_double),
                ("B", C.c_int32), ("T", C.c_int32), ("K", C.c_int32)]


class Embed(C.Structure):
    _fields_ = [("table", _f), ("ids", _f), ("out", _f), ("B", C.c_int32), ("F", C.c_int32), ("H", C.c_int32), ("n_embed", C.c_int32)]


class Tf32Split(C.Structure):
    _fields_ = [("w_hi", _f), ("lo", _f), ("n", C.c_int64)]


class Posterior(C.Structure):
    _fields_ = [("params", _f), ("noise", _f), ("mean", _f), ("logvar", _f), ("std", _f), ("z", _f), ("scale", C.c_float),
                ("B", C.c_int32), ("Z", C.c_int32), ("L", C.c_int32)]


class Stage(C.Structure):
    _fields_ = [("x", _f), ("x_dup", _f), ("x0", _f), ("mask", _f), ("q_noise", _f), ("q_coef", _f), ("noise", _f), ("noise_rows", _f),
                ("B", C.c_int32), ("C", C.c_int32), ("L", C.c_int32), ("reserved_", C.c_int32)]


class Plms(C.Structure):
    _fields_ = [("update", DdimUpdate), ("eps", _f), ("e_prime", _f), ("hist", _f), ("x_stash", _f), ("cfg", C.c_int32),
                ("scale", C.c_float)]


class Ddpm(C.Structure):
    _fields_ = [("x", _f), ("x_dup", _f), ("eps", _f), ("pred_x0", _f), ("noise", _f), ("coef", _f), ("step", _f),
                ("T", C.c_int32), ("B", C.c_int32), ("C", C.c_int32), ("L", C.c_int32), ("cfg", C.c_int32), ("scale", C.c_float),
                ("clip", C.c_int32), ("reserved_", C.c_int32)]


class Dpm(C.Structure):
    _fields_ = [("x", _f), ("x_dup", _f), ("eps", _f), ("pred_x0", _f), ("ring", _f), ("coef", _f), ("step", _f),
                ("n", C.c_int32), ("S", C.c_int32), ("cfg", C.c_int32), ("scale", C.c_float)]


class DpmEx(C.Structure):
    _fields_ = [("dpm", Dpm), ("stage", _f), ("start", _f), ("order_coef", _f), ("B", C.c_int32), ("reserved_", C.c_int32)]


class DpmStop(C.Structure):
    _fields_ = [("dpm", Dpm), ("stop", _f), ("B", C.c_int32), ("reserved_", C.c_int32)]


class Unipc(C.Structure):
    _fields_ = [("dpm", Dpm), ("xc", _f), ("corr", _f)]


class UnipcEx(C.Structure):
    _fields_ = [("unipc", Unipc), ("stage", _f), ("start", _f), ("order_coef", _f), ("order_corr", _f), ("B", C.c_int32),
                ("reserved_", C.c_int32)]


class UnipcStop(C.Structure):
    _fields_ = [("unipc", Unipc), ("stop", _f), ("B", C.c_int32), ("reserved_", C.c_int32)]


class QEncode(C.Structure):
    _fields_ = [("x0", _f), ("noise", _f), ("t", _f), ("sqrt_a", _f), ("sqrt_1ma", _f), ("out", _f),
                ("B", C.c_int32), ("C", C.c_int32), ("L", C.c_int32), ("n", C.c_int32)]


class Join(C.Structure):
    _fields_ = [("x", _f), ("x_dup", _f), ("x_latent", _f), ("join", _f),
                ("B", C.c_int32), ("C", C.c_int32), ("L", C.c_int32), ("reserved_", C.c_int32)]


class Normal(C.Structure):
    _fields_ = [("out", _f), ("seeds", _f), ("n", C.c_int64), ("B", C.c_int32), ("purpose", C.c_int32), ("first_draw", C.c_int32),
                ("n_draws", C.c_int32), ("draw_stride", C.c_int32), ("reserved_", C.c_int32)]


class GroupNormVar(C.Structure):
    _fields_ = [("gn", GroupNorm), ("valid", _f)]


class AttentionVar(C.Structure):
    _fields_ = [("attn", Attention), ("valid", _f)]


class RowMask(C.Structure):
    _fields_ = [("x", _f), ("ld", C.c_int64), ("valid", _f), ("B", C.c_int32), ("L", C.c_int32), ("cols", C.c_int32),
                ("reserved_", C.c_int32)]


class _OpU(C.Union):
    _fields_ = [("gemm", Gemm), ("gn", GroupNorm), ("ln", LayerNorm), ("attn", Attention), ("s4", S4Conv),
                ("ddim", DdimUpdate), ("tr", Transpose), ("cp", Copy2D), ("adv", StepAdvance), ("notes", Notes), ("embed", Embed),
                ("split", Tf32Split), ("post", Posterior), ("gnv", GroupNormVar), ("attnv", AttentionVar), ("mask", RowMask)]


class Op(C.Structure):
    _fields_ = [("kind", C.c_int32), ("tag", C.c_int32), ("u", _OpU)]


_KIND_FIELD = {OP_GEMM: "gemm", OP_GROUPNORM: "gn", OP_LAYERNORM: "ln", OP_ATTENTION: "attn", OP_S4CONV: "s4",
               OP_DDIM_UPDATE: "ddim", OP_TRANSPOSE: "tr", OP_COPY2D: "cp", OP_STEP_ADVANCE: "adv", OP_NOTES: "notes", OP_EMBED: "embed", OP_TF32_SPLIT: "split",
               OP_POSTERIOR: "post", OP_GROUPNORM_VAR: "gnv", OP_ATTENTION_VAR: "attnv", OP_ROW_MASK: "mask"}


def make_op(kind: int, desc, tag: int = 0) -> Op:
    op = Op()
    op.kind = kind
    op.tag = tag
    setattr(op.u, _KIND_FIELD[kind], desc)
    return op


class Region(C.Structure):
    _fields_ = [("name", C.c_char_p), ("base", _f), ("bytes", C.c_int64)]


class MugdError(RuntimeError):
    pass


_lib: Optional[C.CDLL] = None


def load() -> C.CDLL:
    global _lib
    if _lib is not None:
        return _lib
    if not os.path.exists(LIB_PATH):
        raise MugdError(f"{LIB_PATH} not found: build it with `python -m mug_diffusion_b200.build` "
                        "(there is no CPU/PyTorch fallback for the sampler path)")
    lib = C.CDLL(LIB_PATH)
    lib.mugd_last_error.restype = C.c_char_p
    lib.mugd_abi_version.restype = C.c_int
    lib.mugd_create.argtypes = [C.c_int, C.POINTER(C.c_void_p)]
    lib.mugd_destroy.argtypes = [C.c_void_p]
    lib.mugd_destroy.restype = None
    lib.mugd_device_info.argtypes = [C.c_void_p, C.POINTER(C.c_int32), C.POINTER(C.c_int32), C.POINTER(C.c_int32)]
    lib.mugd_set_gemm_impl.argtypes = [C.c_void_p, C.c_int]
    lib.mugd_op_run.argtypes = [C.c_void_p, C.POINTER(Op), C.c_void_p]
    lib.mugd_plan_create.argtypes = [C.c_void_p, C.POINTER(Op), C.c_int32, C.POINTER(C.c_void_p)]
    lib.mugd_plan_run.argtypes = [C.c_void_p, C.c_void_p]
    lib.mugd_plan_capture.argtypes = [C.c_void_p, C.c_void_p]
    lib.mugd_plan_replay.argtypes = [C.c_void_p, C.c_int32, C.c_void_p]
    lib.mugd_plan_launch_count.argtypes = [C.c_void_p]
    lib.mugd_plan_destroy.argtypes = [C.c_void_p]
    lib.mugd_plan_destroy.restype = None
    lib.mugd_s4_kernel_gen.argtypes = [C.c_void_p] + [C.c_void_p] * 7 + [C.c_int32] * 4 + [C.c_void_p, C.c_void_p, C.c_int64, C.c_void_p]
    lib.mugd_melspec.argtypes = [C.c_void_p, C.c_void_p, C.c_int64, C.c_int64, C.c_int32, C.c_void_p, C.c_void_p, C.c_int32,
                                 C.POINTER(C.c_int32), C.POINTER(C.c_int32), C.c_void_p, C.c_int32, C.c_int32,
                                 C.c_void_p, C.c_int64, C.c_int32, C.c_void_p]
    lib.mugd_grid_scan.argtypes = [C.c_void_p, C.c_void_p, C.c_void_p, C.c_int32, C.c_void_p, C.c_int32] + [C.c_void_p] * 11
    lib.mugd_chart_snap.argtypes = [C.c_void_p, C.c_void_p, C.c_void_p, C.c_int32] + [C.c_void_p] * 5
    lib.mugd_remove_mini_jacks.argtypes = [C.c_void_p, C.c_void_p, C.c_int32, C.c_double] + [C.c_void_p] * 7
    lib.mugd_gemm_tc_variant.argtypes =[C.POINTER(Gemm), C.c_int32, C.POINTER(C.c_int32), C.POINTER(C.c_int32), C.POINTER(C.c_int32)]
    lib.mugd_gemm_tc_query.argtypes = [C.c_void_p, C.POINTER(Gemm), C.c_int32, C.POINTER(C.c_int32), C.POINTER(C.c_int32),
                                       C.POINTER(C.c_int64), C.POINTER(C.c_int32)]
    lib.mugd_set_pdl.argtypes = [C.c_int]
    lib.mugd_debug_set_tc_timing.argtypes = [C.c_void_p]
    lib.mugd_fill_i32.argtypes = [C.c_void_p, C.c_int32, C.c_void_p]
    lib.mugd_abi_sizes.argtypes = [C.POINTER(C.c_int32), C.c_int32]
    if lib.mugd_abi_version() != ABI_VERSION:
        raise MugdError(f"libmugd ABI {lib.mugd_abi_version()} != binding {ABI_VERSION}: rebuild the library")
    sizes = (C.c_int32 * 16)()
    lib.mugd_abi_sizes(sizes, 16)
    mine = [C.sizeof(t) for t in (Op, Gemm, GroupNorm, LayerNorm, Attention, S4Conv, DdimUpdate, Transpose, Copy2D, Notes, Embed, Tf32Split,
                                  Posterior, GroupNormVar, AttentionVar, RowMask)]
    if list(sizes) != mine:
        raise MugdError(f"struct layout mismatch: C {list(sizes)} vs ctypes {mine}")
    lib.mugd_sample.argtypes = [C.c_void_p, C.POINTER(Op), C.c_int32, C.c_int32, C.c_void_p]
    lib.mugd_sample_staged.argtypes = [C.c_void_p, C.POINTER(Stage), C.POINTER(Op), C.c_int32, C.c_int32, C.c_void_p]
    lib.mugd_sample_plms.argtypes = [C.c_void_p, C.POINTER(Plms), C.c_int32, C.c_int32, C.c_void_p]
    lib.mugd_plms_combine.argtypes = [C.POINTER(Plms), C.c_int32, C.c_int32, C.c_void_p]
    lib.mugd_sample_ddpm.argtypes = [C.c_void_p, C.POINTER(Ddpm), C.c_int32, C.c_int32, C.c_void_p]
    lib.mugd_ddpm_update.argtypes = [C.POINTER(Ddpm), C.c_void_p]
    lib.mugd_sample_dpm.argtypes = [C.c_void_p, C.POINTER(Dpm), C.c_int32, C.c_int32, C.c_void_p]
    lib.mugd_dpm_update.argtypes = [C.POINTER(Dpm), C.c_void_p]
    lib.mugd_sample_dpm_ex.argtypes = [C.c_void_p, C.POINTER(DpmEx), C.c_int32, C.c_int32, C.c_void_p]
    lib.mugd_dpm_ex_update.argtypes = [C.POINTER(DpmEx), C.c_void_p]
    lib.mugd_sample_dpm_stop.argtypes = [C.c_void_p, C.POINTER(DpmStop), C.c_int32, C.c_int32, C.c_void_p]
    lib.mugd_dpm_stop_update.argtypes = [C.POINTER(DpmStop), C.c_void_p]
    lib.mugd_sample_unipc.argtypes = [C.c_void_p, C.POINTER(Unipc), C.c_int32, C.c_int32, C.c_void_p]
    lib.mugd_unipc_update.argtypes = [C.POINTER(Unipc), C.c_void_p]
    lib.mugd_sample_unipc_ex.argtypes = [C.c_void_p, C.POINTER(UnipcEx), C.c_int32, C.c_int32, C.c_void_p]
    lib.mugd_unipc_ex_update.argtypes = [C.POINTER(UnipcEx), C.c_void_p]
    lib.mugd_sample_unipc_stop.argtypes = [C.c_void_p, C.POINTER(UnipcStop), C.c_int32, C.c_int32, C.c_void_p]
    lib.mugd_unipc_stop_update.argtypes = [C.POINTER(UnipcStop), C.c_void_p]
    lib.mugd_stochastic_encode.argtypes = [C.POINTER(QEncode), C.c_void_p]
    lib.mugd_randn.argtypes = [C.POINTER(Normal), C.c_void_p]
    lib.mugd_sample_join.argtypes = [C.c_void_p, C.POINTER(Join), C.POINTER(Op), C.c_int32, C.c_int32, C.c_int32, C.c_void_p]
    lib.mugd_plan_save.argtypes = [C.c_void_p, C.POINTER(Region), C.c_int32, C.c_char_p]
    lib.mugd_plan_load.argtypes = [C.c_void_p, C.c_char_p, C.POINTER(Region), C.c_int32, C.POINTER(C.c_void_p)]
    lib.mugd_set_tc_single_pass_tf32.argtypes = [C.c_void_p, C.c_int]
    lib.mugd_set_attention_impl.argtypes = [C.c_void_p, C.c_int]
    lib.mugd_set_s4conv_impl.argtypes = [C.c_void_p, C.c_int]
    lib.mugd_debug_set_tc_tile_n.argtypes = [C.c_int]
    lib.mugd_debug_set_tc_cost.argtypes = [C.c_float, C.c_float, C.c_float, C.c_float]
    if os.environ.get("MUGD_TC_COST"):
        lib.mugd_debug_set_tc_cost(*([float(v) for v in os.environ["MUGD_TC_COST"].split(",")] + [0.0] * 4)[:4])
    if os.environ.get("MUGD_TC_TILE"):
        lib.mugd_debug_set_tc_tile_n(int(os.environ["MUGD_TC_TILE"]))
    if os.environ.get("MUGD_TC_BN"):
        lib.mugd_debug_set_tc_tile_n(int(os.environ["MUGD_TC_BN"]))
    if os.environ.get("MUGD_PDL") in ("0", "1"):
        lib.mugd_set_pdl(int(os.environ["MUGD_PDL"]))
    _lib = lib
    return lib


def check(rc: int, what: str = ""):
    if rc != 0:
        msg = load().mugd_last_error().decode(errors="replace")
        if rc == 4:
            import torch
            raise torch.cuda.OutOfMemoryError(f"{what}: {msg}")
        raise MugdError(f"{what} failed (status {rc}): {msg}")


EXPORTED_SYMBOLS = [
    "mugd_abi_version", "mugd_last_error", "mugd_create", "mugd_destroy", "mugd_device_info", "mugd_set_gemm_impl",
    "mugd_op_run", "mugd_plan_create", "mugd_plan_run", "mugd_plan_capture", "mugd_plan_replay",
    "mugd_plan_launch_count", "mugd_plan_destroy", "mugd_s4_kernel_gen", "mugd_fill_i32", "mugd_abi_sizes", "mugd_gemm_tc_query",
    "mugd_set_pdl", "mugd_set_tc_single_pass_tf32", "mugd_set_attention_impl", "mugd_set_s4conv_impl", "mugd_debug_set_tc_tile_n", "mugd_debug_set_tc_cost", "mugd_gemm_tc_variant",
    "mugd_debug_set_attention_dump", "mugd_debug_set_tc_timing", "mugd_sample", "mugd_plan_save", "mugd_plan_load", "mugd_plan_regions", "mugd_plan_ops",
    "mugd_melspec", "mugd_grid_scan", "mugd_chart_snap", "mugd_remove_mini_jacks",
    "mugd_sample_staged", "mugd_sample_plms", "mugd_plms_combine",
    "mugd_sample_ddpm", "mugd_ddpm_update", "mugd_stochastic_encode", "mugd_sample_join",
    "mugd_sample_dpm", "mugd_dpm_update", "mugd_sample_dpm_ex", "mugd_dpm_ex_update",
    "mugd_sample_dpm_stop", "mugd_dpm_stop_update",
    "mugd_sample_unipc", "mugd_unipc_update", "mugd_sample_unipc_ex", "mugd_unipc_ex_update",
    "mugd_sample_unipc_stop", "mugd_unipc_stop_update", "mugd_randn",
]
```

mug_diffusion_b200/netspec.py:

```python
from __future__ import annotations

from dataclasses import dataclass, field
from typing import Dict, Iterator, List, Optional, Tuple

from .config import DecoderConfig, EncoderConfig, UNetConfig


@dataclass
class Block:
    kind: str
    prefix: str
    cin: int
    cout: int
    ds: int
    mul: int = 1
    heads: int = 0
    has_skip_conv: bool = False


@dataclass
class UNetLayout:
    input: List[object] = field(default_factory=list)
    middle: List[Block] = field(default_factory=list)
    output: List[object] = field(default_factory=list)
    out: Optional[Block] = None
    skip_channels: List[int] = field(default_factory=list)

    def blocks(self) -> Iterator[Block]:
        for entry in self.input + [self.middle] + self.output:
            if not isinstance(entry, tuple):
                yield from entry
        yield self.out


RES_LAYERS = {"res": ("in_layers.0.", "in_layers.2.", "out_layers.0.", "out_layers.3.", "skip_connection."),
              "dec_res": ("norm1.", "conv1.", "norm2.", "conv2.", "nin_shortcut.")}


def unet_layout(cfg: UNetConfig, prefix: str = "model.unet_model.") -> UNetLayout:
    mc = cfg.model_channels
    lay = UNetLayout()
    lay.input.append([Block("conv_in", f"{prefix}input_blocks.0.0.", cfg.in_channels, mc, 1)])
    chans = [mc]
    ch, ds, idx = mc, 1, 1
    for level, mult in enumerate(cfg.channel_mult):
        lay.input.append(("audio", level))
        idx += 1
        ch += cfg.audio_channels[level]
        for _ in range(cfg.num_res_blocks):
            cout = mult * mc
            p = f"{prefix}input_blocks.{idx}."
            blocks = [Block("res", p + "0.", ch, cout, ds, has_skip_conv=(ch != cout))]
            ch = cout
            j = 1
            if ds in cfg.attention_resolutions:
                blocks.append(Block("attn", f"{p}{j}.", ch, ch, ds, heads=cfg.num_heads))
                j += 1
            if cfg.s4_layer:
                blocks.append(Block("s4", f"{p}{j}.", ch, ch, ds))
            lay.input.append(blocks)
            chans.append(ch)
            idx += 1
        if level != cfg.levels - 1:
            lay.input.append([Block("down", f"{prefix}input_blocks.{idx}.0.", ch, ch, ds)])
            chans.append(ch)
            idx += 1
            ds *= 2
    lay.skip_channels = list(chans)
    mp = f"{prefix}middle_block."
    lay.middle = [
        Block("res", mp + "0.", ch, ch, ds),
        Block("attn", mp + "1.", ch, ch, ds, heads=cfg.num_heads),
        Block("res", mp + "2.", ch, ch, ds),
    ]
    idx = 0
    for level in reversed(range(cfg.levels)):
        mult = cfg.channel_mult[level]
        lay.output.append(("audio", level))
        idx += 1
        ch += cfg.audio_channels[level]
        for i in range(cfg.num_res_blocks + 1):
            ich = chans.pop()
            cout = mc * mult
            p = f"{prefix}output_blocks.{idx}."
            blocks = [Block("res", p + "0.", ch + ich, cout, ds, has_skip_conv=(ch + ich != cout))]
            ch = cout
            j = 1
            if ds in cfg.attention_resolutions:
                blocks.append(Block("attn", f"{p}{j}.", ch, ch, ds, heads=cfg.num_heads))
                j += 1
            if cfg.s4_layer and i != cfg.num_res_blocks:
                blocks.append(Block("s4", f"{p}{j}.", ch, ch, ds))
                j += 1
            if level and i == cfg.num_res_blocks:
                blocks.append(Block("up", f"{p}{j}.", ch, ch, ds))
                ds //= 2
            lay.output.append(blocks)
            idx += 1
    lay.out = Block("out", f"{prefix}out.", mc, cfg.out_channels, 1)
    return lay


def decoder_layout(cfg: DecoderConfig, prefix: str = "model.first_stage_model.decoder.") -> List[Block]:
    nres = len(cfg.channel_mult)
    block_in = cfg.middle_channels * cfg.channel_mult[-1]
    seq = [Block("dec_conv_in", prefix + "conv_in.", cfg.z_channels, block_in, 1, mul=1)]
    seq.append(Block("dec_res", prefix + "mid.block_1.", block_in, block_in, 1, mul=1))
    seq.append(Block("dec_res", prefix + "mid.block_2.", block_in, block_in, 1, mul=1))
    mul = 1
    for lvl in reversed(range(nres)):
        block_out = cfg.middle_channels * cfg.channel_mult[lvl]
        for b in range(cfg.num_res_blocks + 1):
            seq.append(Block("dec_res", f"{prefix}up.{lvl}.block.{b}.", block_in, block_out, 1, mul=mul,
                             has_skip_conv=(block_in != block_out)))
            block_in = block_out
        if lvl != 0:
            seq.append(Block("up", f"{prefix}up.{lvl}.upsample.", block_in, block_in, 1, mul=mul))
            mul *= 2
    seq.append(Block("dec_out", prefix, block_in, cfg.x_channels, 1, mul=mul))
    return seq


def encoder_layout(cfg: EncoderConfig, prefix: str = "model.first_stage_model.encoder.") -> List[Block]:
    nres = len(cfg.channel_mult)
    mc = cfg.middle_channels
    mul = 1 << (nres - 1)
    seq = [Block("dec_conv_in", prefix + "conv_in.", cfg.x_channels, mc, 1, mul=mul)]
    block_in = mc
    for lvl in range(nres):
        block_out = mc * cfg.channel_mult[lvl]
        for b in range(cfg.num_res_blocks):
            seq.append(Block("dec_res", f"{prefix}down.{lvl}.block.{b}.", block_in, block_out, 1, mul=mul,
                             has_skip_conv=(block_in != block_out)))
            block_in = block_out
        if lvl != nres - 1:
            seq.append(Block("down", f"{prefix}down.{lvl}.downsample.", block_in, block_in, 1, mul=mul))
            mul //= 2
    seq.append(Block("dec_res", prefix + "mid.block_1.", block_in, block_in, 1, mul=mul))
    seq.append(Block("dec_res", prefix + "mid.block_2.", block_in, block_in, 1, mul=mul))
    seq.append(Block("dec_out", prefix, block_in, 2 * cfg.z_channels, 1, mul=mul))
    return seq


Spec = Tuple[Tuple[int, ...], str]


def _conv(out: Dict[str, Spec], pre: str, cin: int, cout: int, k: int):
    out[pre + "weight"] = ((cout, cin, k), "w")
    out[pre + "bias"] = ((cout,), "b")


def _lin(out: Dict[str, Spec], pre: str, cin: int, cout: int, bias: bool = True):
    out[pre + "weight"] = ((cout, cin), "w")
    if bias:
        out[pre + "bias"] = ((cout,), "b")


def _norm(out: Dict[str, Spec], pre: str, c: int):
    out[pre + "weight"] = ((c,), "gamma")
    out[pre + "bias"] = ((c,), "beta")


def _block_params(out: Dict[str, Spec], b: Block, cfg: UNetConfig):
    p = b.prefix
    if b.kind == "conv_in":
        _conv(out, p, b.cin, b.cout, 3)
    elif b.kind == "res":
        _norm(out, p + "in_layers.0.", b.cin)
        _conv(out, p + "in_layers.2.", b.cin, b.cout, 3)
        _lin(out, p + "emb_layers.1.", cfg.time_embed_dim, b.cout)
        _norm(out, p + "out_layers.0.", b.cout)
        _conv(out, p + "out_layers.3.", b.cout, b.cout, 3)
        if b.has_skip_conv:
            _conv(out, p + "skip_connection.", b.cin, b.cout, 1)
    elif b.kind == "attn":
        c = b.cin
        _norm(out, p + "norm.", c)
        _conv(out, p + "proj_in.", c, c, 1)
        t = p + "transformer_blocks.0."
        for name, ctx in (("attn1.", c), ("attn2.", cfg.context_dim)):
            a = t + name
            out[a + "relative_position_embedding"] = ((2 * cfg.pos_max + 1, b.heads), "relpos")
            out[a + "C_embedding"] = ((2 * cfg.pos_max + 1, b.heads), "cemb")
            _lin(out, a + "to_q.", c, c, bias=False)
            _lin(out, a + "to_k.", ctx, c, bias=False)
# ... 68 lines not shown
```

mug_diffusion_b200/packer.py:

```python
from __future__ import annotations

from dataclasses import dataclass
from typing import Dict, List, Optional, Tuple

import torch

from .config import DecoderConfig, EncoderConfig, UNetConfig
from .netspec import RES_LAYERS, Block, decoder_layout, encoder_layout, unet_layout

ALIGN = 64


@dataclass
class Entry:
    offset: int
    shape: Tuple[int, ...]


class WeightBlob:
    def __init__(self):
        self.entries: Dict[str, Entry] = {}
        self._chunks: List[torch.Tensor] = []
        self._size = 0
        self.meta: Dict[str, object] = {}
        self.data: torch.Tensor | None = None
        self.tc: List[Tuple[str, int, int, int]] = []
        self.tc_lo_numel = 0

    def add(self, name: str, t: torch.Tensor):
        assert name not in self.entries, name
        t = t.detach().to(torch.float32).contiguous().reshape(-1).cpu()
        pad = (-self._size) % ALIGN
        if pad:
            self._chunks.append(torch.zeros(pad))
            self._size += pad
        self.entries[name] = Entry(self._size, tuple(t.shape))
        self._chunks.append(t)
        self._size += t.numel()

    def add_shaped(self, name: str, t: torch.Tensor):
        shape = tuple(t.shape)
        self.add(name, t)
        self.entries[name].shape = shape

    def finalize(self) -> torch.Tensor:
        pad = (-self._size) % ALIGN
        if pad:
            self._chunks.append(torch.zeros(pad))
            self._size += pad
        self.data = torch.cat(self._chunks)
        self._chunks = []
        return self.data

    @property
    def numel(self) -> int:
        return self._size

    def offset(self, name: str) -> int:
        return self.entries[name].offset

    def view(self, name: str) -> torch.Tensor:
        e = self.entries[name]
        n = 1
        for s in e.shape:
            n *= s
        return self.data[e.offset:e.offset + n].view(e.shape)


def tf32_rna(x: torch.Tensor) -> torch.Tensor:
    u = x.contiguous().view(torch.int32)
    return ((u + 0x1000) & ~0x1FFF).view(torch.float32)


def tf32_split(w: torch.Tensor):
    hi = tf32_rna(w)
    lo = tf32_rna(w - hi)
    return hi, lo


def _conv3(w: torch.Tensor) -> torch.Tensor:
    return w.permute(0, 2, 1).contiguous().reshape(w.shape[0], -1)


def _conv1(w: torch.Tensor) -> torch.Tensor:
    return w.reshape(w.shape[0], w.shape[1])


def _interleave_halves(w: torch.Tensor) -> torch.Tensor:
    h = w.shape[0] // 2
    return torch.stack([w[:h], w[h:]], dim=1).reshape(w.shape)

# ... 34 lines not shown
            blob.add_shaped(t + a + "C_embedding", sd[t + a + "C_embedding"])
        blob.add_shaped(t + "ff.net.0.proj.weight", _interleave_halves(sd[t + "ff.net.0.proj.weight"]))
        blob.add_shaped(t + "ff.net.0.proj.bias", _interleave_halves(sd[t + "ff.net.0.proj.bias"]))
        for n in ("norm1.", "norm2.", "norm3."):
            blob.add_shaped(t + n + "weight", sd[t + n + "weight"])
            blob.add_shaped(t + n + "bias", sd[t + n + "bias"])
        for norm, lin, wkey, bkey in (("norm1.", "attn1.qkv", t + "attn1.qkv.weight", None),
                                      ("norm2.", "attn2.to_q", t + "attn2.to_q.weight", None),
                                      ("norm3.", "ff.net.0.proj", t + "ff.net.0.proj.weight", t + "ff.net.0.proj.bias")):
            w = blob_tensor(blob, wkey).double()
            gam, bet = sd[t + norm + "weight"].double(), sd[t + norm + "bias"].double()
            wg = (w * gam[None, :]).float()
            blob.add_shaped(t + lin + "_ln.weight", wg)
            blob.add_shaped(t + lin + "_ln.colsum", wg.double().sum(dim=1).float())
            bias = w @ bet + (blob_tensor(blob, bkey).double() if bkey else 0.0)
            blob.add_shaped(t + lin + "_ln.bias", bias.float())
    elif b.kind == "s4":
        blob.add_shaped(p + "norm.weight", sd[p + "norm.weight"])
        blob.add_shaped(p + "norm.bias", sd[p + "norm.bias"])
        s = p + "s4_model."
        blob.add_shaped(s + "D", sd[s + "D"].reshape(-1))
        k = s + "kernel.kernel."
        for n in ("C", "log_dt", "B", "P", "inv_w_real", "w_imag"):
            blob.add_shaped(k + n, sd[k + n])
        blob.meta[k + "L"] = int(sd[k + "L"].item())
        blob.add_shaped(s + "output_linear.0.weight", _interleave_halves(_conv1(sd[s + "output_linear.0.weight"])))
        blob.add_shaped(s + "output_linear.0.bias", _interleave_halves(sd[s + "output_linear.0.bias"]))
        blob.add_shaped(p + "out_layer.weight", _conv3(sd[p + "out_layer.weight"]))
        blob.add_shaped(p + "out_layer.bias", sd[p + "out_layer.bias"])
    elif b.kind in ("down", "up"):
        w = sd[p + "conv.weight"]
        blob.add_shaped(p + "conv.weight", _conv3(w))
        blob.add_shaped(p + "conv.bias", sd[p + "conv.bias"])
        if b.kind == "up":
            w0, w1, w2 = w[:, :, 0], w[:, :, 1], w[:, :, 2]
            blob.add_shaped(p + "conv.up_even.weight", torch.cat([w0, w1 + w2], dim=1).contiguous())
            blob.add_shaped(p + "conv.up_odd.weight", torch.cat([w0 + w1, w2], dim=1).contiguous())
    elif b.kind == "out":
        blob.add_shaped(p + "0.weight", sd[p + "0.weight"])
        blob.add_shaped(p + "0.bias", sd[p + "0.bias"])
        blob.add_shaped(p + "2.weight", _conv3(sd[p + "2.weight"]))
        blob.add_shaped(p + "2.bias", sd[p + "2.bias"])
    elif b.kind == "dec_out":
        blob.add_shaped(p + "norm_out.weight", sd[p + "norm_out.weight"])
        blob.add_shaped(p + "norm_out.bias", sd[p + "norm_out.bias"])
        blob.add_shaped(p + "conv_out.weight", _conv3(sd[p + "conv_out.weight"]))
        blob.add_shaped(p + "conv_out.bias", sd[p + "conv_out.bias"])
    else:
        raise ValueError(b.kind)


def pack_model(sd: Dict[str, torch.Tensor], ucfg: UNetConfig, dcfg: DecoderConfig,
               unet_prefix: str = "model.unet_model.", dec_prefix: str = "model.first_stage_model.decoder.",
               tensor_core_split: bool = True, wave_cfg=None, encoder_cfg: Optional[EncoderConfig] = None,
               enc_prefix: str = "model.first_stage_model.encoder.") -> WeightBlob:
    blob = WeightBlob()
    up = unet_prefix
    for n in ("time_embed.0.", "time_embed.2."):
        blob.add_shaped(up + n + "weight", sd[up + n + "weight"])
        blob.add_shaped(up + n + "bias", sd[up + n + "bias"])
    blocks = list(unet_layout(ucfg, up).blocks())
    res = [b for b in blocks if b.kind == "res"]
    blob.add_shaped(up + "emb_all.weight", torch.cat([sd[b.prefix + "emb_layers.1.weight"] for b in res], dim=0))
    blob.add_shaped(up + "emb_all.bias", torch.cat([sd[b.prefix + "emb_layers.1.bias"] for b in res], dim=0))
    off = 0
    emb_off = {}
    for b in res:
        emb_off[b.prefix] = off
        off += b.cout
    blob.meta["emb_offsets"] = emb_off
    blob.meta["emb_total"] = off
    for b in blocks:
        _pack_block(blob, sd, b)
    for b in decoder_layout(dcfg, dec_prefix):
        _pack_block(blob, sd, b)
    if any(k.startswith(enc_prefix) for k in sd):
        ecfg = encoder_cfg or EncoderConfig()
        for b in encoder_layout(ecfg, enc_prefix):
            _pack_block(blob, sd, b)
        blob.meta["encoder_cfg"] = ecfg
    if wave_cfg is not None or any(k.startswith("model.wave_model.") for k in sd):
        from .wave import WaveConfig, pack_wave
        pack_wave(blob, sd, wave_cfg or WaveConfig())
    blob.tc = []
    lo = 0
    for name in list(blob.entries):
        e = blob.entries[name]
        if tensor_core_split and name.endswith("weight") and len(e.shape) == 2 and e.shape[0] >= 16 and e.shape[1] % 32 == 0:
            n = e.shape[0] * e.shape[1]
            blob.tc.append((name, e.offset, n, lo))
            lo += (n + ALIGN - 1) // ALIGN * ALIGN
    blob.tc_lo_numel = lo
    blob.finalize()
    return blob


def blob_tensor(blob: WeightBlob, name: str) -> torch.Tensor:
    return _chunk_of(blob, name).view(blob.entries[name].shape)


def _chunk_of(blob: WeightBlob, name: str) -> torch.Tensor:
    off = 0
    target = blob.entries[name].offset
    for c in blob._chunks:
        if off == target and c.numel() == int(torch.tensor(blob.entries[name].shape).prod()):
            return c
        off += c.numel()
    raise KeyError(name)
```

mug_diffusion_b200/runtime.py:

```python
from __future__ import annotations

import ctypes as C
import threading
from collections import OrderedDict
from typing import Callable, Dict, List, Optional, Sequence, Tuple

import numpy as np
import torch
from torch.utils.weak import WeakIdKeyDictionary

from . import lib as L_
from .audio import check_z_length
from .config import EncoderConfig, ModelConfig
from .engine import (Arena, CTX_TOKENS_MAX, DecoderCompiler, EncoderCompiler, MAX_STEPS, OpList, UNetCompiler, View, tc_weight_map)
from .packer import WeightBlob, pack_model


def _ptr(t: torch.Tensor) -> int:
    return t.data_ptr()


def _stream() -> int:
    return torch.cuda.current_stream().cuda_stream


class Plan:
    def __init__(self, engine: "MugEngine", ops: OpList):
        self.engine = engine
        self.n_ops = len(ops.ops)
        engine.attach_workspace(ops)
        self._arr = ops.array()
        self.handle = C.c_void_p()
        L_.check(engine.lib.mugd_plan_create(engine.handle, self._arr, self.n_ops, C.byref(self.handle)), "plan_create")
        self.captured = False
        self.launches = 0

    def run(self):
        L_.check(self.engine.lib.mugd_plan_run(self.handle, _stream()), "plan_run")
        self.launches = self.engine.lib.mugd_plan_launch_count(self.handle)

    def capture(self):
        side = torch.cuda.Stream()
        side.wait_stream(torch.cuda.current_stream())
        with torch.cuda.stream(side):
            L_.check(self.engine.lib.mugd_plan_capture(self.handle, side.cuda_stream), "plan_capture")
        torch.cuda.current_stream().wait_stream(side)
        self.launches = self.engine.lib.mugd_plan_launch_count(self.handle)
        self.captured = True

    def replay(self, times: int = 1):
        L_.check(self.engine.lib.mugd_plan_replay(self.handle, times, _stream()), "plan_replay")

    def ensure_captured(self):
        if not self.captured:
            self.run()
            self.capture()

    def _launch_steps(self, entry: str, desc, first_step: int, steps: int):
        self.ensure_captured()
        L_.check(getattr(self.engine.lib, entry)(self.handle, C.byref(desc), first_step, steps, _stream()), entry)

    def launch_plms(self, plms: L_.Plms, first_step: int, steps: int):
        self._launch_steps("mugd_sample_plms", plms, first_step, steps)

    def launch_ddpm(self, ddpm: L_.Ddpm, first_step: int, steps: int):
        self._launch_steps("mugd_sample_ddpm", ddpm, first_step, steps)

    def launch_dpm(self, dpm: L_.Dpm, first_step: int, steps: int):
        self._launch_steps("mugd_sample_dpm", dpm, first_step, steps)

    def launch_dpm_ex(self, ex: L_.DpmEx, first_step: int, steps: int):
        self._launch_steps("mugd_sample_dpm_ex", ex, first_step, steps)

    def launch_dpm_stop(self, e: L_.DpmStop, first_step: int, steps: int):
        self._launch_steps("mugd_sample_dpm_stop", e, first_step, steps)

    def launch_unipc(self, u: L_.Unipc, first_step: int, steps: int):
        self._launch_steps("mugd_sample_unipc", u, first_step, steps)

    def launch_unipc_ex(self, ex: L_.UnipcEx, first_step: int, steps: int):
        self._launch_steps("mugd_sample_unipc_ex", ex, first_step, steps)

    def launch_unipc_stop(self, e: L_.UnipcStop, first_step: int, steps: int):
        self._launch_steps("mugd_sample_unipc_stop", e, first_step, steps)

    def launch_join(self, join: L_.Join, tail: OpList, first_step: int, steps: int):
        self.ensure_captured()
        self.engine.attach_workspace(tail)
        L_.check(self.engine.lib.mugd_sample_join(self.handle, C.byref(join), tail.array(), len(tail.ops), first_step, steps, _stream()),
                 "mugd_sample_join")

    def launch(self, steps: int = 1, tail: Optional[OpList] = None, stage: Optional[L_.Stage] = None):
        self.ensure_captured()
        if tail is None:
            self.replay(steps)
            return
        self.engine.attach_workspace(tail)
        if stage is None:
            L_.check(self.engine.lib.mugd_sample(self.handle, tail.array(), len(tail.ops), steps, _stream()), "mugd_sample")
        else:
            L_.check(self.engine.lib.mugd_sample_staged(self.handle, C.byref(stage), tail.array(), len(tail.ops), steps, _stream()),
                     "mugd_sample_staged")

    def __del__(self):
        try:
            if self.handle:
                self.engine.lib.mugd_plan_destroy(self.handle)
        except Exception:
            pass


def compile_sized(engine: "MugEngine", compile_fn: Callable[[Arena], dict]):
    dry = Arena(0)
    compile_fn(dry)
    nbytes = dry.high + 1024
    arena_t = torch.zeros(nbytes // 4 + 64, device=engine.device)
    base = (arena_t.data_ptr() + 255) // 256 * 256
    res = compile_fn(Arena(base, nbytes))
    return arena_t, res, Plan(engine, res["ops"])


_SPLIT_LO = WeakIdKeyDictionary()


class MugEngine:

    def __init__(self, state_dict: Dict[str, torch.Tensor], cfg: Optional[ModelConfig] = None,
                 device: Optional[torch.device] = None, gemm_impl: str = "auto", blob: Optional[WeightBlob] = None,
                 max_sessions: int = 4, fold_ln: Optional[bool] = None):
        if not torch.cuda.is_available():
            raise L_.MugdError("mug_diffusion_b200 needs an sm_90 (H100) GPU; there is no CPU fallback")
        self.cfg = cfg or ModelConfig()
        self.device = torch.device(device if device is not None else f"cuda:{torch.cuda.current_device()}")
        torch.cuda.set_device(self.device)
        self.lib = L_.load()
        self.handle = C.c_void_p()
        L_.check(self.lib.mugd_create(self.device.index or 0, C.byref(self.handle)), "mugd_create")
        self.blob = blob if blob is not None else pack_model(state_dict, self.cfg.unet, self.cfg.decoder, encoder_cfg=self.cfg.encoder)
        self.weights = self.blob.data.to(self.device)
        self.wbase = self.weights.data_ptr()
        self.weights_lo: Optional[torch.Tensor] = None
        self.tc_split_done = False
        self.tc_map: Dict[int, Tuple[int, int]] = {}
        self.lock = threading.RLock()
        self.tc_ws = torch.zeros(8 * 1024 * 1024, device=self.device)
        self.tc_counters = torch.zeros(4096, dtype=torch.int32, device=self.device)
        self.sessions: "OrderedDict[tuple, Session]" = OrderedDict()
        self.dec_sessions: "OrderedDict[tuple, object]" = OrderedDict()
        self.max_sessions = max_sessions
        self.fold_ln = fold_ln
        self.s4_L: Dict[str, int] = {k: int(v) for k, v in self.blob.meta.items() if k.endswith("kernel.kernel.L")}
        self.set_gemm_impl(gemm_impl)

    def set_gemm_impl(self, impl: str):
        code = {"auto": L_.GEMM_TC, "simt": L_.GEMM_SIMT, "tc": L_.GEMM_TC, "tc_tf32": L_.GEMM_TC}[impl]
        L_.check(self.lib.mugd_set_gemm_impl(self.handle, code), "set_gemm_impl")
        if impl == "simt":
            if self.tc_split_done:
                if self.blob.data.device.type != "cpu":
                    raise L_.MugdError("this engine's weights were split in place and no host copy exists: build a new engine for gemm_impl='simt'")
                self.weights.copy_(self.blob.data)
                self.tc_split_done = False
            self.tc_map = {}
        else:
            self._split_tc_weights()
            self.tc_map = tc_weight_map(self.blob, self.wbase, self.weights_lo.data_ptr())
        L_.check(self.lib.mugd_set_tc_single_pass_tf32(self.handle, 1 if impl == "tc_tf32" else 0), "set_tc_single_pass_tf32")
        self.gemm_impl = impl
        self.sessions.clear()
        self.dec_sessions.clear()

    def _split_tc_weights(self):
        if self.tc_split_done:
            return
        if self.weights in _SPLIT_LO:
            self.weights_lo, self.tc_split_done = _SPLIT_LO[self.weights], True
            return
        if self.weights_lo is None:
            self.weights_lo = torch.zeros(max(self.blob.tc_lo_numel, 4), device=self.device)
        if self.weights is self.blob.data:
            _SPLIT_LO[self.weights] = self.weights_lo
        ops = OpList()
        for _, off, n, lo in self.blob.tc:
            d = L_.Tf32Split()
            d.w_hi, d.lo, d.n = self.wbase + 4 * off, self.weights_lo.data_ptr() + 4 * lo, n
            ops.add(L_.OP_TF32_SPLIT, d)
        st = _stream()
        for op in ops.ops:
            L_.check(self.lib.mugd_op_run(self.handle, C.byref(op), st), "tf32_split")
        self.tc_split_done = True

    def attach_workspace(self, ops: OpList):
        for op in ops.ops:
            if op.kind == L_.OP_GEMM:
                g = op.u.gemm
                g.workspace, g.workspace_bytes = self.tc_ws.data_ptr(), self.tc_ws.numel() * 4
                g.counters, g.n_counters = self.tc_counters.data_ptr(), self.tc_counters.numel()

    def run_ops(self, ops: OpList):
        self.attach_workspace(ops)
        st = _stream()
        for op in ops.ops:
            L_.check(self.lib.mugd_op_run(self.handle, C.byref(op), st), f"op kind {op.kind}")

    def ncl_to_rows(self, x: torch.Tensor, rows: View):
        B, Cc, Lr = x.shape
        ops = OpList()
        ops.transpose(_ptr(x), rows.ptr, 0, rows.ld, B, Cc, Lr, True)
        self.run_ops(ops)

    def rows_to_ncl(self, rows: View, B: int, Cc: int, Lr: int) -> torch.Tensor:
        out = torch.empty(B, Cc, Lr, device=self.device)
        ops = OpList()
        ops.transpose(rows.ptr, _ptr(out), rows.ld, 0, B, Cc, Lr, False)
        self.run_ops(ops)
        return out

    def _lru_get(self, cache: OrderedDict, key, make):
        s = cache.get(key)
        if s is None:
            while len(cache) >= max(1, self.max_sessions):
                _, old = cache.popitem(last=False)
                if hasattr(old, "release"):
                    old.release()
                del old
            s = make()
            cache[key] = s
        else:
            cache.move_to_end(key)
        return s

    def session(self, Beff: int, Lz: int, per_sample_t: bool = False, ragged: bool = False) -> "Session":
        check_z_length(Lz)
        if not ragged:
            return self._lru_get(self.sessions, (Beff, Lz, per_sample_t), lambda: Session(self, Beff, Lz, per_sample_t))
        return self._lru_get(self.sessions, (Beff, Lz, per_sample_t, "ragged"), lambda: Session(self, Beff, Lz, per_sample_t, ragged=True))

    def wave_session(self, B: int, T: int):
        if "wave_cfg" not in self.blob.meta:
            raise L_.MugdError("this engine was packed without model.wave_model.* weights")
        from .wave import WaveSession
        return self._lru_get(self.dec_sessions, ("wave", B, T), lambda: WaveSession(self, B, T))

    def decoder_session(self, B: int, Lz: int, ragged: bool = False) -> "DecoderSession":
        check_z_length(Lz)
        if not ragged:
            return self._lru_get(self.dec_sessions, (B, Lz), lambda: DecoderSession(self, B, Lz))
        return self._lru_get(self.dec_sessions, (B, Lz, "ragged"), lambda: DecoderSession(self, B, Lz, ragged=True))

    @property
    def encoder_cfg(self) -> EncoderConfig:
        if "encoder_cfg" not in self.blob.meta:
            raise L_.MugdError("this engine was packed without model.first_stage_model.encoder.* weights")
        return self.blob.meta["encoder_cfg"]

    def encoder_session(self, B: int, Lz: int) -> "EncoderSession":
        self.encoder_cfg
        return self._lru_get(self.dec_sessions, ("enc", B, Lz), lambda: EncoderSession(self, B, Lz))

    def __del__(self):
        try:
            self.sessions.clear()
            self.dec_sessions.clear()
            if self.handle:
                self.lib.mugd_destroy(self.handle)
        except Exception:
            pass


class Session:

    def __init__(self, engine: MugEngine, Beff: int, Lz: int, per_sample_t: bool, ragged: bool = False):
        self.engine, self.Beff, self.Lz, self.per_sample_t = engine, Beff, Lz, per_sample_t
        cfg = engine.cfg.unet
        dev = engine.device
        self.valid = torch.tensor([[Lz >> l] * Beff for l in range(cfg.levels)], dtype=torch.int32, device=dev) if ragged else None
        self.lens: Optional[List[int]] = None
        self.comp = UNetCompiler(cfg, engine.blob, engine.wbase, engine.tc_map)
        emb_total = engine.blob.meta["emb_total"]
        attn_blocks = [b for b in self.comp.lay.blocks() if b.kind == "attn"]
        s4b = [b for b in self.comp.lay.blocks() if b.kind == "s4"]

        emb_rows = Beff if per_sample_t else MAX_STEPS
        self.emb_table = torch.zeros(emb_rows, emb_total, device=dev)
        self.temb = torch.zeros(emb_rows, cfg.model_channels, device=dev)
        self.emb_h1 = torch.zeros(emb_rows, cfg.time_embed_dim, device=dev)
        self.emb_h2 = torch.zeros(emb_rows, cfg.time_embed_dim, device=dev)
        self.step = torch.zeros(1, dtype=torch.int32, device=dev)
        self.coef = torch.zeros(MAX_STEPS, 4, device=dev)
        self.ctx = torch.zeros(Beff * CTX_TOKENS_MAX, cfg.context_dim, device=dev)
        self.ctx_kv = [torch.zeros(Beff * CTX_TOKENS_MAX, 2 * b.cin, device=dev) for b in attn_blocks]
        self.ctx_tokens = 21
        self.s4_kt = {b.prefix: torch.zeros(Lz // b.ds, b.cin, device=dev) for b in s4b}
        self._gen_s4_kernels(s4b)
        self._build()

    def _gen_s4_kernels(self, s4b):
        eng = self.engine
        N = eng.cfg.unet.s4_state // 2
        ws = None
        for b in s4b:
            k = b.prefix + "s4_model.kernel.kernel."
            L_int = int(eng.s4_L[k + "L"])
            L_req = self.Lz // b.ds
            if L_req > L_int:
                from . import s4_setup

                def grab(n):
                    e = eng.blob.entries[k + n]
                    cnt = int(np.prod(e.shape))
                    return eng.weights[e.offset:e.offset + cnt].view(e.shape).detach().cpu()

                params = {n: grab(n) for n in ("C", "log_dt", "P", "inv_w_real", "w_imag")}
                C_new, L_int = s4_setup.lengthen(params, L_int, L_req)
                e = eng.blob.entries[k + "C"]
                eng.weights[e.offset:e.offset + C_new.numel()].copy_(C_new.reshape(-1).to(eng.device))
                eng.s4_L[k + "L"] = L_int
            need = 16 * b.cin * (L_int // 2 + 1)
            if ws is None or ws.numel() * 8 < need:
                ws = torch.empty(need // 8 + 2, dtype=torch.float64, device=eng.device)

            def w(n):
                return eng.wbase + 4 * eng.blob.offset(k + n)

            om = s4_fft_nodes(L_int).to(eng.device)
            L_.check(eng.lib.mugd_s4_kernel_gen(eng.handle, w("log_dt"), w("B"), w("C"), w("P"), w("inv_w_real"), w("w_imag"),
                                                _ptr(om), b.cin, N, L_int, L_req, _ptr(self.s4_kt[b.prefix]), _ptr(ws), ws.numel() * 8,
                                                _stream()), "s4_kernel_gen")
        torch.cuda.current_stream().synchronize()

    def _ext(self, base_ctx_tokens: int) -> dict:
        return dict(
            emb_table=_ptr(self.emb_table), step=_ptr(self.step), ctx_tokens=base_ctx_tokens,
            ctx_kv=[View(_ptr(t), t.shape[1], self.Beff * base_ctx_tokens, t.shape[1]) for t in self.ctx_kv],
            s4_kt={p: View(_ptr(t), t.shape[1], t.shape[0], t.shape[1]) for p, t in self.s4_kt.items()},
        )

    def _build(self):
        fold = False if self.engine.gemm_impl == "simt" else self.engine.fold_ln
        valid = None if self.valid is None else [_ptr(self.valid[l]) for l in range(self.valid.shape[0])]
        self.arena_t, res, self.plan = compile_sized(self.engine, lambda arena: self.comp.compile(
            arena, self.Beff, self.Lz, self._ext(self.ctx_tokens), self.per_sample_t, fold, valid))
        self.xin: View = res["xin"]
        self.eps: View = res["eps"]
        self.audio_slots = res["audio_slots"]
        self.ln_folded = res["ln_folded"]

    def set_ctx_tokens(self, T: int):
        if T != self.ctx_tokens:
            self.ctx_tokens = T
            self._build()

    def set_lengths(self, lens: Sequence[int]):
        assert self.valid is not None, "set_lengths needs a ragged session"
        lens = [int(v) for v in lens]
        assert len(lens) == self.Beff and all(32 <= v <= self.Lz and v % 32 == 0 for v in lens), lens
        t = torch.tensor([[v >> l for v in lens] for l in range(self.valid.shape[0])], dtype=torch.int32)
        self.valid.copy_(t.to(self.engine.device))
        self.lens = lens

    def set_timestep_table(self, timesteps: Sequence[int]):
        cfg = self.engine.cfg.unet
        eng = self.engine
        ts = np.asarray(timesteps)
        if ts.dtype.kind == "f":
            t = torch.as_tensor(ts.astype(np.float32))
        else:
            t = torch.as_tensor(ts, dtype=torch.long)
        R = t.shape[0]
        assert R <= self.temb.shape[0]
        half = cfg.model_channels // 2
        import math
        freqs = torch.exp(-math.log(10000.0) * torch.arange(0, half, dtype=torch.float32) / half)
        args = t[:, None].float() * freqs[None]
        emb = torch.cat([torch.cos(args), torch.sin(args)], dim=-1)
        self.temb[:R].copy_(emb.to(eng.device))
        eng.run_ops(self.timestep_ops(R))

    def timestep_ops(self, R: int) -> OpList:
        cfg = self.engine.cfg.unet
        eng = self.engine
        ops = OpList(eng.tc_map)
        up = self.comp.prefix
        tv = View(_ptr(self.temb), cfg.model_channels, R, cfg.model_channels)
        h1 = View(_ptr(self.emb_h1), cfg.time_embed_dim, R, cfg.time_embed_dim)
        h2 = View(_ptr(self.emb_h2), cfg.time_embed_dim, R, cfg.time_embed_dim)
        et = View(_ptr(self.emb_table), self.emb_table.shape[1], R, self.emb_table.shape[1])
        w = self.comp.w
        ops.gemm(tv, w(up + "time_embed.0.weight"), cfg.time_embed_dim, cfg.model_channels, h1, bias=w(up + "time_embed.0.bias"),
                 act=L_.ACT_SILU)
        ops.gemm(h1, w(up + "time_embed.2.weight"), cfg.time_embed_dim, cfg.time_embed_dim, h2, bias=w(up + "time_embed.2.bias"),
                 act=L_.ACT_SILU)
        ops.gemm(h2, w(up + "emb_all.weight"), self.emb_table.shape[1], cfg.time_embed_dim, et, bias=w(up + "emb_all.bias"))
        return ops

    def set_context(self, context):
        eng = self.engine
        cfg = eng.cfg.unet
        parts = list(context) if isinstance(context, (list, tuple)) else [context]
        parts = [c.to(eng.device, torch.float32).contiguous() for c in parts]
        Bc = sum(int(c.shape[0]) for c in parts)
        _, Cd, T = parts[0].shape
        assert Bc == self.Beff and Cd == cfg.context_dim and T <= CTX_TOKENS_MAX and all(c.shape[1:] == parts[0].shape[1:] for c in parts)
        self.set_ctx_tokens(T)
        eng.run_ops(self.context_ops([(_ptr(c), int(c.shape[0])) for c in parts], T))
        self._keep = parts

    def context_ops(self, parts: Sequence, T: int) -> OpList:
        eng = self.engine
        cfg = eng.cfg.unet
        Cd = cfg.context_dim
        Bc = sum(b for _, b in parts)
        ops = OpList(eng.tc_map)
        row = 0
        for addr, bpart in parts:
            ops.transpose(addr, _ptr(self.ctx) + 4 * row * Cd, 0, Cd, bpart, Cd, T, True)
            row += bpart * T
        cv = View(_ptr(self.ctx), Cd, Bc * T, Cd)
        blocks = [b for b in self.comp.lay.blocks() if b.kind == "attn"]
        for b, kv in zip(blocks, self.ctx_kv):
            o = View(_ptr(kv), kv.shape[1], Bc * T, kv.shape[1])
            ops.gemm(cv, self.comp.w(b.prefix + "transformer_blocks.0.attn2.kv.weight"), 2 * b.cin, Cd, o, Lout=T)
        return ops

    def set_audio(self, audios: Sequence[torch.Tensor], dup: bool = False):
        cfg = self.engine.cfg.unet
        w4 = [a.to(self.engine.device, torch.float32).contiguous() for a in list(audios)[-cfg.levels:]]
        Bh = self.Beff // 2 if dup else self.Beff
        for lvl in range(cfg.levels):
            assert w4[lvl].shape == (Bh, cfg.audio_channels[lvl], self.Lz >> lvl), (w4[lvl].shape, lvl)
        self.engine.run_ops(self.audio_ops([_ptr(a) for a in w4], dup))
        self._keep_audio = w4

    def audio_ops(self, addrs: Sequence[int], dup: bool) -> OpList:
        cfg = self.engine.cfg.unet
        Bh = self.Beff // 2 if dup else self.Beff
        ops = OpList()
        for lvl, view in self.audio_slots:
            Cc, Lr = cfg.audio_channels[lvl], self.Lz >> lvl
            ops.transpose(addrs[lvl], view.ptr, 0, view.ld, Bh, Cc, Lr, True)
            if dup:
                ops.transpose(addrs[lvl], view.r(Bh * Lr, 2 * Bh * Lr).ptr, 0, view.ld, Bh, Cc, Lr, True)
        return ops

    def load_x(self, x: torch.Tensor, dup: bool):
        x = x.to(self.engine.device, torch.float32).contiguous()
        B, Cc, Lr = x.shape
        self.engine.run_ops(self.loadx_ops(_ptr(x), B, dup))
        self._keep_x = x

    def loadx_ops(self, addr: int, B: int, dup: bool) -> OpList:
        Cc, Lr = self.engine.cfg.unet.in_channels, self.Lz
        ops = OpList()
        ops.transpose(addr, self.xin.ptr, 0, self.xin.ld, B, Cc, Lr, True)
        if dup:
            ops.transpose(addr, self.xin.r(B * Lr, 2 * B * Lr).ptr, 0, self.xin.ld, B, Cc, Lr, True)
        return ops

    def read_rows(self, view: View, B: int, Cc: int, Lr: int) -> torch.Tensor:
        return self.engine.rows_to_ncl(view, B, Cc, Lr)

    def eval(self, graph: bool = True):
        if graph:
            self.plan.launch()
        else:
            self.plan.run()

    def set_ddim_schedule(self, alphas, alphas_prev, sigmas, sqrt_one_minus_alphas):
        coef = np.stack([np.asarray(a, dtype=np.float32) for a in (alphas, alphas_prev, sigmas, sqrt_one_minus_alphas)], axis=1)
        self.coef.zero_()
        self.coef[:len(coef)].copy_(torch.from_numpy(coef).to(self.engine.device))

    def _x_rows(self, B: int, cfg_on: bool):
        return self.xin.ptr, (self.xin.r(B * self.Lz, 2 * B * self.Lz).ptr if cfg_on else None)

    def ddim_update(self, B: int, S: int, cfg_on: bool, scale: float, temperature: float, pred_x0: int, noise: int = 0) -> L_.DdimUpdate:
        n = B * self.Lz * self.engine.cfg.unet.in_channels
        upd = L_.DdimUpdate()
        upd.x, upd.x_dup = self._x_rows(B, cfg_on)
        upd.eps, upd.noise, upd.pred_x0 = self.eps.ptr, noise or None, pred_x0
        upd.coef, upd.step = _ptr(self.coef), _ptr(self.step)
        upd.S, upd.n, upd.cfg, upd.scale, upd.temperature = S, n, int(cfg_on), float(scale), float(temperature)
        return upd

    def plms(self, B: int, S: int, cfg_on: bool, scale: float, pred_x0: int, work: torch.Tensor) -> L_.Plms:
        n = B * self.Lz * self.engine.cfg.unet.in_channels
        assert work.shape == (5, n) and work.dtype == torch.float32 and work.is_contiguous()
        p = L_.Plms()
        p.update = self.ddim_update(B, S, cfg_on, 1.0, 1.0, pred_x0)
        p.update.cfg, p.update.eps = 0, _ptr(work[0])
        p.eps, p.e_prime, p.hist, p.x_stash = self.eps.ptr, _ptr(work[0]), _ptr(work[1]), _ptr(work[4])
        p.cfg, p.scale = int(cfg_on), float(scale)
        return p

    def ddpm(self, B: int, T: int, cfg_on: bool, scale: float, clip: bool, pred_x0: int, noise: int, coef: torch.Tensor) -> L_.Ddpm:
        assert coef.shape == (T, 5) and coef.dtype == torch.float32 and coef.is_contiguous()
        d = L_.Ddpm()
        d.x, d.x_dup = self._x_rows(B, cfg_on)
        d.eps, d.pred_x0, d.noise, d.coef, d.step = self.eps.ptr, pred_x0 or None, noise, _ptr(coef), _ptr(self.step)
        d.T, d.B, d.C, d.L = T, B, self.engine.cfg.unet.in_channels, self.Lz
        d.cfg, d.scale, d.clip = int(cfg_on), float(scale), int(bool(clip))
        return d

    def dpm(self, B: int, S: int, cfg_on: bool, scale: float, pred_x0: int, ring: torch.Tensor, coef: torch.Tensor) -> L_.Dpm:
        n = B * self.Lz * self.engine.cfg.unet.in_channels
        assert coef.shape == (S, 8) and coef.dtype == torch.float32 and coef.is_contiguous()
        assert ring.shape == (3, n) and ring.dtype == torch.float32 and ring.is_contiguous()
        d = L_.Dpm()
        d.x, d.x_dup = self._x_rows(B, cfg_on)
        d.eps, d.pred_x0, d.ring, d.coef, d.step = self.eps.ptr, pred_x0 or None, _ptr(ring), _ptr(coef), _ptr(self.step)
        d.n, d.S, d.cfg, d.scale = n, S, int(cfg_on), float(scale)
        return d

    def dpm_ex(self, dpm: L_.Dpm, stage: Optional[L_.Stage] = None, B: int = 0, start: Optional[torch.Tensor] = None,
               order_coef: Optional[torch.Tensor] = None) -> L_.DpmEx:
        e = L_.DpmEx()
        e.dpm = dpm
        e.stage = C.addressof(stage) if stage is not None else None
        if start is not None:
            assert start.shape == (B,) and start.dtype == torch.int32 and start.is_contiguous()
            assert order_coef.shape == (dpm.S, 3, 8) and order_coef.dtype == torch.float32 and order_coef.is_contiguous()
            e.start, e.order_coef, e.B = _ptr(start), _ptr(order_coef), B
        return e

    def dpm_stop(self, dpm: L_.Dpm, B: int, stop: torch.Tensor) -> L_.DpmStop:
# ... 193 lines not shown
```

Baseline: 244.1.

## Hoist audio-conditioning channels of res-block convs out of the denoising loop

The audio channels concatenated into res blocks stay fixed across denoising steps. This change splits the first conv and skip-conv weights so their audio-only contribution is computed once when audio is loaded (hoist ops), and per-step GEMMs cover only the varying channels. A new gap-aware groupnorm kernel skips writing the hoisted channel range. The tensor-core split heuristic is also tweaked. This adds weight repacking, extra buffers and bundle tensors, and makes the setup path more complex.

```diff
diff --git a/include/mugd.h b/include/mugd.h
--- a/include/mugd.h
+++ b/include/mugd.h
@@ -172,6 +172,11 @@
     int32_t B, L, cols, reserved_;
 } mugd_row_mask;
 
+typedef struct mugd_groupnorm_gap {
+    mugd_groupnorm_var gnv;
+    int32_t gap0, gap1;
+} mugd_groupnorm_gap;
+
 typedef struct mugd_op {
     int32_t kind;
     int32_t tag;
@@ -180,6 +185,7 @@
         mugd_ddim_update ddim; mugd_transpose tr; mugd_copy2d cp; mugd_step_advance adv; mugd_notes notes;
         mugd_embed embed; mugd_tf32_split split; mugd_posterior post;
         mugd_groupnorm_var gnv; mugd_attention_var attnv; mugd_row_mask mask;
+        mugd_groupnorm_gap gng;
     } u;
 } mugd_op;
 
diff --git a/mug_diffusion_b200/bundle.py b/mug_diffusion_b200/bundle.py
--- a/mug_diffusion_b200/bundle.py
+++ b/mug_diffusion_b200/bundle.py
@@ -77,7 +77,8 @@
         sess.set_timestep_table(ts.copy())
         sess.set_ddim_schedule(sampler.ddim_alphas, sampler.ddim_alphas_prev, sampler.ddim_sigmas, sampler.ddim_sqrt_one_minus_alphas)
 
-        tensors: Dict[str, torch.Tensor] = dict(weights=eng.weights, weights_lo=eng.weights_lo, arena=sess.arena_t, emb_table=sess.emb_table, temb=sess.temb,
+        tensors: Dict[str, torch.Tensor] = dict(weights=eng.weights, weights_lo=eng.weights_lo, weights_hoist=eng.weights_hoist,
+                                                weights_hoist_lo=eng.weights_hoist_lo, arena=sess.arena_t, emb_table=sess.emb_table, temb=sess.temb,
                                                 emb_h1=sess.emb_h1, emb_h2=sess.emb_h2, step=sess.step, coef=sess.coef, ctx=sess.ctx,
                                                 tc_ws=eng.tc_ws, tc_counters=eng.tc_counters, dec_arena=dec.arena_t)
         for i, t in enumerate(sess.ctx_kv):
@@ -85,7 +86,7 @@
         for i, (_, t) in enumerate(sorted(sess.s4_kt.items())):
             tensors[f"s4_kt{i}"] = t
         tensors.update(st)
-        contents = {"weights", "weights_lo", "temb", "coef"} | {k for k in tensors if k.startswith("s4_kt")}
+        contents = {"weights", "weights_lo", "weights_hoist", "weights_hoist_lo", "temb", "coef"} | {k for k in tensors if k.startswith("s4_kt")}
         inputs = {k for k in st if k.startswith("in_")}
         names = list(tensors)
         keep = [n.encode() for n in names]
diff --git a/mug_diffusion_b200/csrc/api.cu b/mug_diffusion_b200/csrc/api.cu
--- a/mug_diffusion_b200/csrc/api.cu
+++ b/mug_diffusion_b200/csrc/api.cu
@@ -40,7 +40,9 @@
 static int dispatch(mugd_handle* h, const mugd_op& op, cudaStream_t st, int* launches, const mugd_gemm* next_tc = nullptr) {
     switch (op.kind) {
         case MUGD_OP_GEMM: return launch_gemm(h->dev, op.u.gemm, h->default_gemm_impl, next_tc, st, launches);
-        case MUGD_OP_GROUPNORM: return launch_groupnorm(h->dev, op.u.gn, st, launches);
+        case MUGD_OP_GROUPNORM:
+            if (op.u.gng.gap0 != op.u.gng.gap1) return launch_groupnorm_gap(h->dev, op.u.gn, nullptr, op.u.gng.gap0, op.u.gng.gap1, st, launches);
+            return launch_groupnorm(h->dev, op.u.gn, st, launches);
         case MUGD_OP_LAYERNORM: return launch_layernorm(h->dev, op.u.ln, st, launches);
         case MUGD_OP_ATTENTION: return launch_attention(h->dev, op.u.attn, st, launches);
         case MUGD_OP_S4CONV: return launch_s4conv(h->dev, op.u.s4, st, launches);
@@ -52,7 +54,12 @@
         case MUGD_OP_EMBED: return launch_embed(h->dev, op.u.embed, st, launches);
         case MUGD_OP_TF32_SPLIT: return launch_tf32_split(h->dev, op.u.split, st, launches);
         case MUGD_OP_POSTERIOR: return launch_posterior(h->dev, op.u.post, st, launches);
-        case MUGD_OP_GROUPNORM_VAR: return launch_groupnorm_var(h->dev, op.u.gnv, st, launches);
+        case MUGD_OP_GROUPNORM_VAR:
+            if (op.u.gng.gap0 != op.u.gng.gap1) {
+                MUGD_REQUIRE(op.u.gnv.valid, "groupnorm_var: valid lengths missing");
+                return launch_groupnorm_gap(h->dev, op.u.gnv.gn, op.u.gnv.valid, op.u.gng.gap0, op.u.gng.gap1, st, launches);
+            }
+            return launch_groupnorm_var(h->dev, op.u.gnv, st, launches);
         case MUGD_OP_ATTENTION_VAR: return launch_attention_var(h->dev, op.u.attnv, st, launches);
         case MUGD_OP_ROW_MASK: return launch_row_mask(h->dev, op.u.mask, st, launches);
         default:
@@ -415,6 +422,7 @@
     out[9] = sizeof(mugd_notes); out[10] = sizeof(mugd_embed); out[11] = sizeof(mugd_tf32_split);
     out[12] = sizeof(mugd_posterior);
     if (n >= 16) { out[13] = sizeof(mugd_groupnorm_var); out[14] = sizeof(mugd_attention_var); out[15] = sizeof(mugd_row_mask); }
+    if (n >= 17) out[16] = sizeof(mugd_groupnorm_gap);
     return MUGD_OK;
 }
 
diff --git a/mug_diffusion_b200/csrc/common.cuh b/mug_diffusion_b200/csrc/common.cuh
--- a/mug_diffusion_b200/csrc/common.cuh
+++ b/mug_diffusion_b200/csrc/common.cuh
@@ -59,6 +59,8 @@
 int launch_tf32_split(const DeviceInfo& dev, const mugd_tf32_split& s, cudaStream_t st, int* launches);
 int launch_posterior(const DeviceInfo& dev, const mugd_posterior& p, cudaStream_t st, int* launches);
 int launch_groupnorm_var(const DeviceInfo& dev, const mugd_groupnorm_var& g, cudaStream_t st, int* launches);
+int launch_groupnorm_gap(const DeviceInfo& dev, const mugd_groupnorm& g, const int32_t* valid, int gap0, int gap1, cudaStream_t st,
+                         int* launches);
 int launch_attention_var(const DeviceInfo& dev, const mugd_attention_var& a, cudaStream_t st, int* launches);
 int launch_row_mask(const DeviceInfo& dev, const mugd_row_mask& m, cudaStream_t st, int* launches);
 int check_stage(const mugd_stage& s, int32_t n_steps);
diff --git a/mug_diffusion_b200/csrc/gemm_tc.cu b/mug_diffusion_b200/csrc/gemm_tc.cu
--- a/mug_diffusion_b200/csrc/gemm_tc.cu
+++ b/mug_diffusion_b200/csrc/gemm_tc.cu
@@ -98,7 +98,7 @@
         const int sp_max = forced_split > 0 ? forced_split : (tiles < sm_count ? 16 : 1);
         for (int sp = forced_split > 0 ? forced_split : 1; sp <= sp_max && sp <= h.total_it; ++sp) {
             const int per = (h.total_it + sp - 1) / sp;
-            if (forced_split <= 0 && sp > 1 && per < 2) break;
+            if (forced_split <= 0 && sp > 1 && h.total_it / sp < 2) break;
             if (forced_split <= 0 && sp > 1 && tiles * sp > 2 * sm_count) break;
             const int waves = (tiles * sp + sm_count - 1) / sm_count;
             const float est = waves * (1.0f + kstep * per) + (sp > 1 ? g_tc_split : 0.0f);
diff --git a/mug_diffusion_b200/csrc/norm.cu b/mug_diffusion_b200/csrc/norm.cu
--- a/mug_diffusion_b200/csrc/norm.cu
+++ b/mug_diffusion_b200/csrc/norm.cu
@@ -24,17 +24,22 @@
     rstd = r;
 }
 
-template <int NV>
+struct GnGap { int gap0, gap1, skip0, nskip; };
+
+__device__ __forceinline__ int gn_group(const GnGap& gp) { return (int)blockIdx.x + ((int)blockIdx.x >= gp.skip0 ? gp.nskip : 0); }
+__device__ __forceinline__ int gn_gap_col(int c, const GnGap& gp) { return c >= gp.gap1 ? c - (gp.gap1 - gp.gap0) : (c >= gp.gap0 ? -1 : c); }
+
+template <int NV, bool GAP = false>
 __device__ __forceinline__ void gn_reg_body(const float* __restrict__ x, int64_t ldx, float* __restrict__ y, int64_t ldy,
                                             const float* __restrict__ gamma, const float* __restrict__ beta,
-                                            int L, int Lv, int C, int G, float eps, int silu) {
-    const int g = blockIdx.x, b = blockIdx.y;
+                                            int L, int Lv, int C, int G, float eps, int silu, GnGap gp = {}) {
+    const int g = GAP ? gn_group(gp) : (int)blockIdx.x, b = blockIdx.y;
     const int cg = C / G;
     const int q = cg >> 2;
     const int total = Lv * q;
     const double inv_n = 1.0 / ((double)Lv * cg);
     const float* xb = x + (int64_t)b * L * ldx + (int64_t)g * cg;
-    float* yb = y + (int64_t)b * L * ldy + (int64_t)g * cg;
+    float* yb = y + (int64_t)b * L * ldy + (GAP ? 0 : (int64_t)g * cg);
     float4 v[NV];
 #pragma unroll
     for (int u = 0; u < NV; ++u) {
@@ -80,7 +85,12 @@
             o.z = (v[u].z - mean) * rstd * ga.z + be.z;
             o.w = (v[u].w - mean) * rstd * ga.w + be.w;
             if (silu) { o.x = silu_f(o.x); o.y = silu_f(o.y); o.z = silu_f(o.z); o.w = silu_f(o.w); }
-            st_f4(yb + (int64_t)row * ldy + qq * 4, o);
+            if constexpr (GAP) {
+                const int col = gn_gap_col(g * cg + qq * 4, gp);
+                if (col >= 0) st_f4(yb + (int64_t)row * ldy + col, o);
+            } else {
+                st_f4(yb + (int64_t)row * ldy + qq * 4, o);
+            }
         }
     }
 }
@@ -94,16 +104,17 @@
     gn_reg_body<NV>(x, ldx, y, ldy, gamma, beta, L, L, C, G, eps, silu);
 }
 
+template <bool GAP = false>
 __device__ __forceinline__ void gn_body(const float* __restrict__ x, int64_t ldx, float* __restrict__ y, int64_t ldy,
                                         const float* __restrict__ gamma, const float* __restrict__ beta,
-                                        int L, int Lv, int C, int G, float eps, int silu) {
-    const int g = blockIdx.x, b = blockIdx.y;
+                                        int L, int Lv, int C, int G, float eps, int silu, GnGap gp = {}) {
+    const int g = GAP ? gn_group(gp) : (int)blockIdx.x, b = blockIdx.y;
     const int cg = C / G;
     const int q = cg >> 2;
     const int total = Lv * q;
     const double inv_n = 1.0 / ((double)Lv * cg);
     const float* xb = x + (int64_t)b * L * ldx + (int64_t)g * cg;
-    float* yb = y + (int64_t)b * L * ldy + (int64_t)g * cg;
+    float* yb = y + (int64_t)b * L * ldy + (GAP ? 0 : (int64_t)g * cg);
 
     double s = 0.0, ss = 0.0;
     for (int i = threadIdx.x; i < total; i += GN_THREADS) {
@@ -127,7 +138,12 @@
         o.z = (v.z - mean) * rstd * ga.z + be.z;
         o.w = (v.w - mean) * rstd * ga.w + be.w;
         if (silu) { o.x = silu_f(o.x); o.y = silu_f(o.y); o.z = silu_f(o.z); o.w = silu_f(o.w); }
-        st_f4(yb + (int64_t)row * ldy + qq * 4, o);
+        if constexpr (GAP) {
+            const int col = gn_gap_col(g * cg + qq * 4, gp);
+            if (col >= 0) st_f4(yb + (int64_t)row * ldy + col, o);
+        } else {
+            st_f4(yb + (int64_t)row * ldy + qq * 4, o);
+        }
     }
 }
 
@@ -141,14 +157,20 @@
 
 __device__ __forceinline__ int gn_valid_rows(const int32_t* valid, int L) { return min(max(valid[blockIdx.y], 0), L); }
 
-__device__ __forceinline__ void gn_zero_tail(float* y, int64_t ldy, int L, int Lv, int C, int G) {
-    const int g = blockIdx.x, b = blockIdx.y;
+template <bool GAP = false>
+__device__ __forceinline__ void gn_zero_tail(float* y, int64_t ldy, int L, int Lv, int C, int G, GnGap gp = {}) {
+    const int g = GAP ? gn_group(gp) : (int)blockIdx.x, b = blockIdx.y;
     const int q = (C / G) >> 2;
-    float* yb = y + ((int64_t)b * L + Lv) * ldy + (int64_t)g * (C / G);
+    float* yb = y + ((int64_t)b * L + Lv) * ldy + (GAP ? 0 : (int64_t)g * (C / G));
     const float4 z = make_float4(0.f, 0.f, 0.f, 0.f);
     for (int i = threadIdx.x; i < (L - Lv) * q; i += GN_THREADS) {
         const int row = i / q, qq = i - row * q;
-        st_f4(yb + (int64_t)row * ldy + qq * 4, z);
+        if constexpr (GAP) {
+            const int col = gn_gap_col(g * (C / G) + qq * 4, gp);
+            if (col >= 0) st_f4(yb + (int64_t)row * ldy + col, z);
+        } else {
+            st_f4(yb + (int64_t)row * ldy + qq * 4, z);
+        }
     }
 }
 
@@ -173,12 +195,33 @@
     gn_zero_tail(y, ldy, L, Lv, C, G);
 }
 
-static int check_groupnorm(const mugd_groupnorm& g) {
+template <int NV>
+__global__ void __launch_bounds__(GN_THREADS)
+groupnorm_silu_reg_gap_kernel(const float* __restrict__ x, int64_t ldx, float* __restrict__ y, int64_t ldy,
+                              const float* __restrict__ gamma, const float* __restrict__ beta,
+                              int L, int C, int G, float eps, int silu, const int32_t* __restrict__ valid, GnGap gp) {
+    pdl_wait();
+    const int Lv = valid ? gn_valid_rows(valid, L) : L;
+    gn_reg_body<NV, true>(x, ldx, y, ldy, gamma, beta, L, Lv, C, G, eps, silu, gp);
+    if (valid) gn_zero_tail<true>(y, ldy, L, Lv, C, G, gp);
+}
+
+__global__ void __launch_bounds__(GN_THREADS)
+groupnorm_silu_gap_kernel(const float* __restrict__ x, int64_t ldx, float* __restrict__ y, int64_t ldy,
+                          const float* __restrict__ gamma, const float* __restrict__ beta,
+                          int L, int C, int G, float eps, int silu, const int32_t* __restrict__ valid, GnGap gp) {
+    pdl_wait();
+    const int Lv = valid ? gn_valid_rows(valid, L) : L;
+    gn_body<true>(x, ldx, y, ldy, gamma, beta, L, Lv, C, G, eps, silu, gp);
+    if (valid) gn_zero_tail<true>(y, ldy, L, Lv, C, G, gp);
+}
+
+static int check_groupnorm(const mugd_groupnorm& g, int gap = 0) {
     MUGD_REQUIRE(g.B > 0 && g.L > 0 && g.C > 0 && g.G > 0, "groupnorm: empty shape B=%d L=%d C=%d G=%d", g.B, g.L, g.C, g.G);
     MUGD_REQUIRE(g.C % g.G == 0 && (g.C / g.G) % 4 == 0, "groupnorm: C/G must be a multiple of 4 (C=%d G=%d)", g.C, g.G);
     MUGD_REQUIRE(g.ldx % 4 == 0 && g.ldy % 4 == 0 && aligned16(g.x) && aligned16(g.y) && aligned16(g.gamma) && aligned16(g.beta),
                  "groupnorm: operands must be 16-byte aligned with ld %% 4 == 0");
-    MUGD_REQUIRE(g.ldx >= g.C && g.ldy >= g.C, "groupnorm: leading dimension smaller than C");
+    MUGD_REQUIRE(g.ldx >= g.C && g.ldy >= g.C - gap, "groupnorm: leading dimension smaller than C");
     return MUGD_OK;
 }
 
@@ -218,6 +261,33 @@
     return MUGD_OK;
 }
 
+int launch_groupnorm_gap(const DeviceInfo&, const mugd_groupnorm& g, const int32_t* valid, int gap0, int gap1, cudaStream_t st,
+                         int* launches) {
+    MUGD_REQUIRE(0 <= gap0 && gap0 < gap1 && gap1 <= g.C && gap0 % 4 == 0 && gap1 % 4 == 0,
+                 "groupnorm: gap [%d, %d) must be a non-empty range of multiples of 4 inside C=%d", gap0, gap1, g.C);
+    const int rc = check_groupnorm(g, gap1 - gap0);
+    if (rc != MUGD_OK) return rc;
+    const int cg = g.C / g.G;
+    GnGap gp;
+    gp.gap0 = gap0;
+    gp.gap1 = gap1;
+    gp.skip0 = (gap0 + cg - 1) / cg;
+    gp.nskip = max(gap1 / cg - gp.skip0, 0);
+    MUGD_REQUIRE(gp.nskip < g.G, "groupnorm: the gap covers every group");
+    dim3 grid(g.G - gp.nskip, g.B);
+    const int per_thread = (g.L * (cg / 4) + GN_THREADS - 1) / GN_THREADS;
+#define GN_GO(K) MUGD_CHECK_CUDA(launch_k(K, grid, dim3(GN_THREADS), 0, st, g.x, g.ldx, g.y, g.ldy, g.gamma, g.beta, g.L, g.C, g.G, g.eps, g.silu, valid, gp))
+    if (per_thread <= 2) GN_GO(groupnorm_silu_reg_gap_kernel<2>);
+    else if (per_thread <= 4) GN_GO(groupnorm_silu_reg_gap_kernel<4>);
+    else if (per_thread <= 8) GN_GO(groupnorm_silu_reg_gap_kernel<8>);
+    else if (per_thread <= 16) GN_GO(groupnorm_silu_reg_gap_kernel<16>);
+    else if (per_thread <= GN_MAXV) GN_GO(groupnorm_silu_reg_gap_kernel<GN_MAXV>);
+    else GN_GO(groupnorm_silu_gap_kernel);
+#undef GN_GO
+    if (launches) *launches += 1;
+    return MUGD_OK;
+}
+
 constexpr int LN_WARPS = 8;
 constexpr int LN_MAXQ = 8;
 
diff --git a/mug_diffusion_b200/engine.py b/mug_diffusion_b200/engine.py
--- a/mug_diffusion_b200/engine.py
+++ b/mug_diffusion_b200/engine.py
@@ -10,7 +10,7 @@
 from . import lib as L_
 from .config import DecoderConfig, EncoderConfig, ModelConfig, UNetConfig
 from .dpm_solver import MAX_STEPS
-from .netspec import RES_LAYERS, Block, decoder_layout, encoder_layout, unet_layout
+from .netspec import RES_LAYERS, AudioHoist, Block, audio_hoist, decoder_layout, encoder_layout, unet_layout
 from .packer import WeightBlob, pack_model
 
 GN_EPS = 1e-6
@@ -115,7 +115,8 @@
         tc = bool(g.W_hi) and g.K % 32 == 0 and g.K2 % 32 == 0 and g.N >= 16 and g.impl != L_.GEMM_SIMT and g.conv_mode != L_.CONV_UP
         return tc and g.act == L_.ACT_NONE and g.gate == L_.GATE_NONE and not g.ln_stats and not g.row_moments
 
-    def groupnorm(self, x: View, y: View, gamma: int, beta: int, B: int, Lrows: int, G: int, silu: bool, tag: int = 0) -> int:
+    def groupnorm(self, x: View, y: View, gamma: int, beta: int, B: int, Lrows: int, G: int, silu: bool, tag: int = 0,
+                  gap: Tuple[int, int] = (0, 0)) -> int:
         d = L_.GroupNorm()
         d.x, d.ldx, d.y, d.ldy = x.ptr, x.ld, y.ptr, y.ld
         d.gamma, d.beta = gamma, beta
@@ -128,6 +129,8 @@
             self.add(L_.OP_GROUPNORM_VAR, v, tag)
         else:
             self.add(L_.OP_GROUPNORM, d, tag)
+        if gap != (0, 0):
+            self.ops[-1].u.gng.gap0, self.ops[-1].u.gng.gap1 = gap
         return len(self.ops) - 1
 
     def row_mask(self, x: View, B: int, Lrows: int, tag: int = 0):
@@ -201,18 +204,37 @@
 TAG_RES, TAG_ATTN, TAG_S4, TAG_UPDOWN, TAG_IO = 1, 2, 3, 4, 5
 
 
-def emit_res(ops: OpList, arena: Arena, wfn, b: Block, x: View, out: View, B: int, Lr: int, G: int, **emb):
+@dataclass
+class HoistedRes:
+    spec: AudioHoist
+    p1: View
+    pskip: Optional[View]
+
+
+def emit_res(ops: OpList, arena: Arena, wfn, b: Block, x: View, out: View, B: int, Lr: int, G: int, hoist: Optional[HoistedRes] = None,
+             **emb):
     norm1, conv1, norm2, conv2, _ = RES_LAYERS[b.kind]
     p = b.prefix
     m = arena.mark()
     t1 = arena.alloc(x.rows, b.cin)
-    ops.groupnorm(x, t1, wfn(p + norm1 + "weight"), wfn(p + norm1 + "bias"), B, Lr, G, True, TAG_RES)
-    t2 = arena.alloc(x.rows, b.cout)
-    ops.gemm(t1, wfn(p + conv1 + "weight"), b.cout, b.cin, t2, bias=wfn(p + conv1 + "bias"), taps=3, mode=L_.CONV_SAME, Lin=Lr, Lout=Lr,
-             tag=TAG_RES, **emb)
+    a = hoist.spec if hoist is not None else None
+    if a is None:
+        ops.groupnorm(x, t1, wfn(p + norm1 + "weight"), wfn(p + norm1 + "bias"), B, Lr, G, True, TAG_RES)
+        t2 = arena.alloc(x.rows, b.cout)
+        ops.gemm(t1, wfn(p + conv1 + "weight"), b.cout, b.cin, t2, bias=wfn(p + conv1 + "bias"), taps=3, mode=L_.CONV_SAME, Lin=Lr,
+                 Lout=Lr, tag=TAG_RES, **emb)
+    else:
+        K = b.cin - (a.S2 - a.S1)
+        ops.groupnorm(x, t1, wfn(p + norm1 + "weight"), wfn(p + norm1 + "bias"), B, Lr, G, True, TAG_RES, gap=(a.S1, a.S2))
+        t2 = arena.alloc(x.rows, b.cout)
+        ops.gemm(t1.c(0, K), wfn(p + conv1 + "step.weight"), b.cout, K, t2, bias=wfn(p + conv1 + "bias"), taps=3, mode=L_.CONV_SAME,
+                 Lin=Lr, Lout=Lr, residual=hoist.p1, tag=TAG_RES, **emb)
     t3 = arena.alloc(x.rows, b.cout)
     ops.groupnorm(t2, t3, wfn(p + norm2 + "weight"), wfn(p + norm2 + "bias"), B, Lr, G, True, TAG_RES)
-    if b.has_skip_conv:
+    if b.has_skip_conv and hoist is not None and hoist.pskip is not None:
+        ops.gemm(t3, wfn(p + "out_skip.step.weight"), b.cout, b.cout, out, bias=wfn(p + "out_skip.bias"), taps=3, mode=L_.CONV_SAME,
+                 Lin=Lr, Lout=Lr, A2=x.c(0, a.h), residual=hoist.pskip, tag=TAG_RES)
+    elif b.has_skip_conv:
         ops.gemm(t3, wfn(p + "out_skip.weight"), b.cout, b.cout, out, bias=wfn(p + "out_skip.bias"), taps=3, mode=L_.CONV_SAME,
                  Lin=Lr, Lout=Lr, A2=x, tag=TAG_RES)
     else:
@@ -224,12 +246,22 @@
 class UNetCompiler:
 
     def __init__(self, cfg: UNetConfig, blob: WeightBlob, wbase: int, tc_map: Optional[Dict[int, Tuple[int, int]]] = None,
-                 prefix: str = "model.unet_model."):
+                 prefix: str = "model.unet_model.", hoist_blob: Optional[WeightBlob] = None, hoist_base: Optional[int] = None):
         self.cfg, self.blob, self.wbase, self.prefix = cfg, blob, wbase, prefix
-        self.tc_map = tc_weight_map(blob, wbase) if tc_map is None else tc_map
+        if hoist_blob is not None and hoist_base is None:
+            hoist_base = wbase + 4 * (blob.numel + blob.tc_lo_numel)
+        self.hoist_blob, self.hoist_base = hoist_blob, hoist_base
+        if tc_map is None:
+            tc_map = tc_weight_map(blob, wbase)
+            if hoist_blob is not None:
+                tc_map.update(tc_weight_map(hoist_blob, hoist_base))
+        self.tc_map = tc_map
         self.lay = unet_layout(cfg, prefix)
+        self.hoist = {a.prefix: a for a in audio_hoist(cfg, prefix)} if hoist_blob is not None else {}
 
     def w(self, name: str) -> int:
+        if self.hoist_blob is not None and name in self.hoist_blob.entries:
+            return self.hoist_base + 4 * self.hoist_blob.offset(name)
         return self.wbase + 4 * self.blob.offset(name)
 
     def compile(self, arena: Arena, Beff: int, Lz: int, ext: Dict[str, int], per_sample_t: bool, fold_ln: Optional[bool] = None,
@@ -307,6 +339,17 @@
             audio_slots.append((level, up_cat[bi].c(ch_h, ch_h + ca)))
             bi += cfg.num_res_blocks + 1
 
+        cat_of: Dict[str, Tuple[int, View]] = {}
+        for i, entry in enumerate(self.lay.input):
+            if isinstance(entry, tuple):
+                cat_of[self.lay.input[i + 1][0].prefix] = (entry[1], down_cat[entry[1]])
+        for bi, blocks in enumerate(up_blocks):
+            cat_of[blocks[0].prefix] = (nlev - 1 - bi // (cfg.num_res_blocks + 1), up_cat[bi])
+        hoisted: Dict[str, HoistedRes] = {}
+        for p, a in self.hoist.items():
+            n = rows[cat_of[p][0]]
+            hoisted[p] = HoistedRes(a, arena.alloc(n, a.cout), arena.alloc(n, a.cout) if a.down and a.has_skip_conv else None)
+
         emb_total = self.blob.meta["emb_total"]
         emb_off = self.blob.meta["emb_offsets"]
         E = ext["emb_table"]
@@ -405,7 +448,8 @@
                     continue
                 out = final_out if (last and final_out is not None) else arena.alloc(cur.rows, b.cout)
                 if b.kind == "res":
-                    emit_res(ops, arena, self.w, b, cur, out, Beff, lens[lvl], G, rowvec=E + 4 * emb_off[b.prefix], **emb_row)
+                    emit_res(ops, arena, self.w, b, cur, out, Beff, lens[lvl], G, hoisted.get(b.prefix), rowvec=E + 4 * emb_off[b.prefix],
+                             **emb_row)
                 elif b.kind == "attn":
                     emit_attn(b, cur, out, lvl)
                 elif b.kind == "s4":
@@ -471,7 +515,26 @@
         gemm(t, self.w(ob.prefix + "2.weight"), ob.cout, ob.cin, eps, bias=self.w(ob.prefix + "2.bias"), taps=3,
              mode=L_.CONV_SAME, Lin=lens[0], Lout=lens[0], tag=TAG_IO)
         arena.release(m)
-        return dict(ops=ops, xin=xin, eps=eps, audio_slots=audio_slots, ln_folded=fuse_ln)
+
+        hoist = OpList(self.tc_map, ops.valid)
+        m = arena.mark()
+        if ragged and hoisted:
+            for l, view in audio_slots:
+                hoist.row_mask(view, Beff, lens[l], TAG_IO)
+        for p, hz in hoisted.items():
+            a = hz.spec
+            lvl_, x = cat_of[p]
+            cg = a.C // G
+            g0, g1 = a.S1 // cg, -(-a.S2 // cg)
+            t = arena.alloc(x.rows, (g1 - g0) * cg)
+            hoist.groupnorm(x.c(g0 * cg, g1 * cg), t, self.w(p + "in_layers.0.weight") + 4 * g0 * cg,
+                            self.w(p + "in_layers.0.bias") + 4 * g0 * cg, Beff, lens[lvl_], g1 - g0, True, TAG_RES)
+            hoist.gemm(t.c(a.S1 - g0 * cg, a.S2 - g0 * cg), self.w(p + "in_layers.2.hoist.weight"), a.cout, a.S2 - a.S1, hz.p1, taps=3,
+                       mode=L_.CONV_SAME, Lin=lens[lvl_], Lout=lens[lvl_], tag=TAG_RES)
+            if hz.pskip is not None:
+                hoist.gemm(x.c(a.h, a.C), self.w(p + "skip_audio.weight"), a.cout, a.audio, hz.pskip, Lout=lens[lvl_], tag=TAG_RES)
+        arena.release(m)
+        return dict(ops=ops, xin=xin, eps=eps, audio_slots=audio_slots, ln_folded=fuse_ln, hoist=hoist)
 
 
 class DecoderCompiler:
diff --git a/mug_diffusion_b200/lib.py b/mug_diffusion_b200/lib.py
--- a/mug_diffusion_b200/lib.py
+++ b/mug_diffusion_b200/lib.py
@@ -155,6 +155,10 @@
     _fields_ = [("gn", GroupNorm), ("valid", _f)]
 
 
+class GroupNormGap(C.Structure):
+    _fields_ = [("gnv", GroupNormVar), ("gap0", C.c_int32), ("gap1", C.c_int32)]
+
+
 class AttentionVar(C.Structure):
     _fields_ = [("attn", Attention), ("valid", _f)]
 
@@ -167,7 +171,8 @@
 class _OpU(C.Union):
     _fields_ = [("gemm", Gemm), ("gn", GroupNorm), ("ln", LayerNorm), ("attn", Attention), ("s4", S4Conv),
                 ("ddim", DdimUpdate), ("tr", Transpose), ("cp", Copy2D), ("adv", StepAdvance), ("notes", Notes), ("embed", Embed),
-                ("split", Tf32Split), ("post", Posterior), ("gnv", GroupNormVar), ("attnv", AttentionVar), ("mask", RowMask)]
+                ("split", Tf32Split), ("post", Posterior), ("gnv", GroupNormVar), ("attnv", AttentionVar), ("mask", RowMask),
+                ("gng", GroupNormGap)]
 
 
 class Op(C.Structure):
@@ -237,10 +242,10 @@
     lib.mugd_abi_sizes.argtypes = [C.POINTER(C.c_int32), C.c_int32]
     if lib.mugd_abi_version() != ABI_VERSION:
         raise MugdError(f"libmugd ABI {lib.mugd_abi_version()} != binding {ABI_VERSION}: rebuild the library")
-    sizes = (C.c_int32 * 16)()
-    lib.mugd_abi_sizes(sizes, 16)
+    sizes = (C.c_int32 * 17)()
+    lib.mugd_abi_sizes(sizes, 17)
     mine = [C.sizeof(t) for t in (Op, Gemm, GroupNorm, LayerNorm, Attention, S4Conv, DdimUpdate, Transpose, Copy2D, Notes, Embed, Tf32Split,
-                                  Posterior, GroupNormVar, AttentionVar, RowMask)]
+                                  Posterior, GroupNormVar, AttentionVar, RowMask, GroupNormGap)]
     if list(sizes) != mine:
         raise MugdError(f"struct layout mismatch: C {list(sizes)} vs ctypes {mine}")
     lib.mugd_sample.argtypes = [C.c_void_p, C.POINTER(Op), C.c_int32, C.c_int32, C.c_void_p]
diff --git a/mug_diffusion_b200/netspec.py b/mug_diffusion_b200/netspec.py
--- a/mug_diffusion_b200/netspec.py
+++ b/mug_diffusion_b200/netspec.py
@@ -101,6 +101,39 @@
     return lay
 
 
+@dataclass
+class AudioHoist:
+    prefix: str
+    h: int
+    audio: int
+    C: int
+    cout: int
+    S1: int
+    S2: int
+    down: bool
+    has_skip_conv: bool
+
+
+def audio_hoist(cfg: UNetConfig, prefix: str = "model.unet_model.") -> List[AudioHoist]:
+    lay = unet_layout(cfg, prefix)
+    out = []
+    for part, down in ((lay.input, True), (lay.output, False)):
+        blocks = 0
+        for i, entry in enumerate(part):
+            if not isinstance(entry, tuple):
+                blocks += 1
+                continue
+            b = part[i + 1][0]
+            a = cfg.audio_channels[entry[1]]
+            h = b.cin - a - (0 if down else lay.skip_channels[-1 - blocks])
+            cg = b.cin // cfg.gn_groups
+            S1 = -(-(-(-h // cg) * cg) // 32) * 32
+            S2 = b.cin if down else ((h + a) // cg * cg) // 32 * 32
+            if S1 < S2:
+                out.append(AudioHoist(b.prefix, h, a, b.cin, b.cout, S1, S2, down, b.has_skip_conv))
+    return out
+
+
 def decoder_layout(cfg: DecoderConfig, prefix: str = "model.first_stage_model.decoder.") -> List[Block]:
     nres = len(cfg.channel_mult)
     block_in = cfg.middle_channels * cfg.channel_mult[-1]
diff --git a/mug_diffusion_b200/packer.py b/mug_diffusion_b200/packer.py
--- a/mug_diffusion_b200/packer.py
+++ b/mug_diffusion_b200/packer.py
@@ -1,12 +1,12 @@
 from __future__ import annotations
 
 from dataclasses import dataclass
-from typing import Dict, List, Optional, Tuple
+from typing import Callable, Dict, List, Optional, Tuple
 
 import torch
 
 from .config import DecoderConfig, EncoderConfig, UNetConfig
-from .netspec import RES_LAYERS, Block, decoder_layout, encoder_layout, unet_layout
+from .netspec import RES_LAYERS, Block, audio_hoist, decoder_layout, encoder_layout, unet_layout
 
 ALIGN = 64
 
@@ -207,6 +207,12 @@
     if wave_cfg is not None or any(k.startswith("model.wave_model.") for k in sd):
         from .wave import WaveConfig, pack_wave
         pack_wave(blob, sd, wave_cfg or WaveConfig())
+    _list_tc(blob, tensor_core_split)
+    blob.finalize()
+    return blob
+
+
+def _list_tc(blob: WeightBlob, tensor_core_split: bool = True):
     blob.tc = []
     lo = 0
     for name in list(blob.entries):
@@ -216,8 +222,25 @@
             blob.tc.append((name, e.offset, n, lo))
             lo += (n + ALIGN - 1) // ALIGN * ALIGN
     blob.tc_lo_numel = lo
-    blob.finalize()
-    return blob
+
+
+def pack_audio_hoist(ucfg: UNetConfig, weight: Optional[Callable[[str], torch.Tensor]] = None,
+                     prefix: str = "model.unet_model.") -> WeightBlob:
+    hb = WeightBlob()
+    for a in audio_hoist(ucfg, prefix):
+        p = a.prefix
+        n3 = 3 * a.cout
+        w1 = weight(p + "in_layers.2.weight") if weight else torch.zeros(a.cout, 3 * a.C)
+        w1 = w1.reshape(a.cout, 3, a.C)
+        hb.add_shaped(p + "in_layers.2.step.weight", torch.cat([w1[:, :, :a.S1], w1[:, :, a.S2:]], dim=2).reshape(a.cout, -1))
+        hb.add_shaped(p + "in_layers.2.hoist.weight", w1[:, :, a.S1:a.S2].reshape(a.cout, -1))
+        if a.down and a.has_skip_conv:
+            ws = weight(p + "out_skip.weight") if weight else torch.zeros(a.cout, n3 + a.C)
+            hb.add_shaped(p + "out_skip.step.weight", ws[:, :n3 + a.h])
+            hb.add_shaped(p + "skip_audio.weight", ws[:, n3 + a.h:])
+    _list_tc(hb)
+    hb.finalize()
+    return hb
 
 
 def blob_tensor(blob: WeightBlob, name: str) -> torch.Tensor:
diff --git a/mug_diffusion_b200/runtime.py b/mug_diffusion_b200/runtime.py
--- a/mug_diffusion_b200/runtime.py
+++ b/mug_diffusion_b200/runtime.py
@@ -13,7 +13,7 @@
 from .audio import check_z_length
 from .config import EncoderConfig, ModelConfig
 from .engine import (Arena, CTX_TOKENS_MAX, DecoderCompiler, EncoderCompiler, MAX_STEPS, OpList, UNetCompiler, View, tc_weight_map)
-from .packer import WeightBlob, pack_model
+from .packer import WeightBlob, pack_audio_hoist, pack_model
 
 
 def _ptr(t: torch.Tensor) -> int:
@@ -140,6 +140,9 @@
         self.weights = self.blob.data.to(self.device)
         self.wbase = self.weights.data_ptr()
         self.weights_lo: Optional[torch.Tensor] = None
+        self.hoist_blob: Optional[WeightBlob] = None
+        self.weights_hoist: Optional[torch.Tensor] = None
+        self.weights_hoist_lo: Optional[torch.Tensor] = None
         self.tc_split_done = False
         self.tc_map: Dict[int, Tuple[int, int]] = {}
         self.lock = threading.RLock()
@@ -161,30 +164,48 @@
                     raise L_.MugdError("this engine's weights were split in place and no host copy exists: build a new engine for gemm_impl='simt'")
                 self.weights.copy_(self.blob.data)
                 self.tc_split_done = False
+            self._cut_hoist_weights()
             self.tc_map = {}
         else:
             self._split_tc_weights()
-            self.tc_map = tc_weight_map(self.blob, self.wbase, self.weights_lo.data_ptr())
+            self.tc_map = {**tc_weight_map(self.blob, self.wbase, self.weights_lo.data_ptr()),
+                           **tc_weight_map(self.hoist_blob, self.weights_hoist.data_ptr(), self.weights_hoist_lo.data_ptr())}
         L_.check(self.lib.mugd_set_tc_single_pass_tf32(self.handle, 1 if impl == "tc_tf32" else 0), "set_tc_single_pass_tf32")
         self.gemm_impl = impl
         self.sessions.clear()
         self.dec_sessions.clear()
 
+    def _cut_hoist_weights(self):
+        def view(name: str) -> torch.Tensor:
+            e = self.blob.entries[name]
+            return self.weights[e.offset:e.offset + int(np.prod(e.shape))].view(e.shape)
+
+        self.hoist_blob = pack_audio_hoist(self.cfg.unet, view)
+        if self.weights_hoist is None:
+            self.weights_hoist = self.hoist_blob.data.to(self.device)
+        else:
+            self.weights_hoist.copy_(self.hoist_blob.data)
+
     def _split_tc_weights(self):
         if self.tc_split_done:
             return
         if self.weights in _SPLIT_LO:
-            self.weights_lo, self.tc_split_done = _SPLIT_LO[self.weights], True
+            self.weights_lo, (self.hoist_blob, self.weights_hoist, self.weights_hoist_lo) = _SPLIT_LO[self.weights]
+            self.tc_split_done = True
             return
+        self._cut_hoist_weights()
         if self.weights_lo is None:
             self.weights_lo = torch.zeros(max(self.blob.tc_lo_numel, 4), device=self.device)
+        if self.weights_hoist_lo is None:
+            self.weights_hoist_lo = torch.zeros(max(self.hoist_blob.tc_lo_numel, 4), device=self.device)
         if self.weights is self.blob.data:
-            _SPLIT_LO[self.weights] = self.weights_lo
+            _SPLIT_LO[self.weights] = (self.weights_lo, (self.hoist_blob, self.weights_hoist, self.weights_hoist_lo))
         ops = OpList()
-        for _, off, n, lo in self.blob.tc:
-            d = L_.Tf32Split()
-            d.w_hi, d.lo, d.n = self.wbase + 4 * off, self.weights_lo.data_ptr() + 4 * lo, n
-            ops.add(L_.OP_TF32_SPLIT, d)
+        for blob, w, lo_buf in ((self.blob, self.weights, self.weights_lo), (self.hoist_blob, self.weights_hoist, self.weights_hoist_lo)):
+            for _, off, n, lo in blob.tc:
+                d = L_.Tf32Split()
+                d.w_hi, d.lo, d.n = w.data_ptr() + 4 * off, lo_buf.data_ptr() + 4 * lo, n
+                ops.add(L_.OP_TF32_SPLIT, d)
         st = _stream()
         for op in ops.ops:
             L_.check(self.lib.mugd_op_run(self.handle, C.byref(op), st), "tf32_split")
@@ -276,7 +297,8 @@
         dev = engine.device
         self.valid = torch.tensor([[Lz >> l] * Beff for l in range(cfg.levels)], dtype=torch.int32, device=dev) if ragged else None
         self.lens: Optional[List[int]] = None
-        self.comp = UNetCompiler(cfg, engine.blob, engine.wbase, engine.tc_map)
+        self.comp = UNetCompiler(cfg, engine.blob, engine.wbase, engine.tc_map, hoist_blob=engine.hoist_blob,
+                                 hoist_base=engine.weights_hoist.data_ptr())
         emb_total = engine.blob.meta["emb_total"]
         attn_blocks = [b for b in self.comp.lay.blocks() if b.kind == "attn"]
         s4b = [b for b in self.comp.lay.blocks() if b.kind == "s4"]
@@ -344,6 +366,7 @@
         self.xin: View = res["xin"]
         self.eps: View = res["eps"]
         self.audio_slots = res["audio_slots"]
+        self.hoist_ops: OpList = res["hoist"]
         self.ln_folded = res["ln_folded"]
 
     def set_ctx_tokens(self, T: int):
@@ -441,6 +464,7 @@
             ops.transpose(addrs[lvl], view.ptr, 0, view.ld, Bh, Cc, Lr, True)
             if dup:
                 ops.transpose(addrs[lvl], view.r(Bh * Lr, 2 * Bh * Lr).ptr, 0, view.ld, Bh, Cc, Lr, True)
+        ops.ops.extend(self.hoist_ops.ops)
         return ops
 
     def load_x(self, x: torch.Tensor, dup: bool):
```

Result: no change. 248.0, median of 6 (+1.6%).
